# aleflabo/MoCoDAD

Hardware: AMD Instinct MI355X
Metric: pose-clips/sec (whole node) @ noise_steps=10, 5 seeds; AUC vs ref (higher is better)
Workload: dtype f32

## Files before the change

### mocodad_amd/csrc/mcd_api.hip

```cpp

#include <algorithm>
#include "mcd_launch.hpp"
#include "mcd_generic_kernel.hpp"
#include "mcd_pack.hpp"

#if MCD_NWAVES != 8 && !defined(MCD_FAST_T)
#error "mcd_api.hip is built with the default wave count: per-unit wave counts belong to mcd_inst.hip (MCD_UNIT_FLAGS_<n>)"
#endif
namespace { constexpr int API_THREADS = 512; }
#pragma GCC poison NWAVES NTHREADS

using namespace mcd;

#include "mcd_post_kernel.hpp"

namespace {

int launch_score(const mcd_weights* w, int T, ScoreParams& P, hipStream_t st, bool* fused = nullptr, bool layer_test = false) {
    if (!layer_test) {
        P.force_split = w->opt[MCD_OPT_SPLIT];
        P.phase = w->opt[MCD_OPT_PHASE];
        const int variant = w->opt[MCD_OPT_VARIANT];
        if (variant != 0 && !score_has_variants()) return fail(MCD_EUNSUPPORTED, "MCD_OPT_VARIANT needs a -DMCD_TUNING_VARIANTS build");
#define MCD_CASE(unit, V, T_, NB, MINW) if (T == T_ && variant == V) return launch_score_t<T_, NB, MINW>(P, st, fused);
        MCD_SCORE_VARIANT_INSTANCES(MCD_CASE)
#undef MCD_CASE
    }
    switch (layer_test ? -T : T) {
#define MCD_CASE(unit, T_, NB, MINW, LT) case (LT ? -T_ : T_): return launch_score_t<T_, NB, MINW, LT>(P, st, fused);
        MCD_SCORE_INSTANCES(MCD_CASE)
#undef MCD_CASE
        default: break;
    }
    if (layer_test) return fail(MCD_EUNSUPPORTED, "mcd_layer_forward: no layer-test kernel for " + std::to_string(T) + " U-Net frames (the LT rows of mcd_instances.hpp)");
    return fail(MCD_EUNSUPPORTED, "U-Net frame count " + std::to_string(T) + " not instantiated (MCD_SCORE_INSTANCES, mcd_instances.hpp)");
}

#define MCD_COND_CASE(fn, unit, T, NB) case T: return fn<T, NB>(w, data, fi, seg_len, emb, B, st);
int launch_cond_fast(const mcd_weights* w, const DataView& data, const FrameIdx& fi, int seg_len, float* emb, int B, hipStream_t st) {
    switch (w->cond.Tc) {
#define MCD_CASE(unit, T, NB) MCD_COND_CASE(launch_cond_fast_t, unit, T, NB)
        MCD_COND_FAST_INSTANCES(MCD_CASE)
#undef MCD_CASE
        default: break;
    }
    return fail(MCD_EUNSUPPORTED, "cond_fast: frame count not instantiated");
}
int launch_cond_unet(const mcd_weights* w, const DataView& data, const FrameIdx& fi, int seg_len, float* emb, int B, hipStream_t st) {
    switch (w->cond.Tc) {
#define MCD_CASE(unit, T, NB) MCD_COND_CASE(launch_cond_unet_t, unit, T, NB)
        MCD_COND_UNET_INSTANCES(MCD_CASE)
#undef MCD_CASE
        default: break;
    }
    return fail(MCD_EUNSUPPORTED, "E_unet condition encoder: frame count not instantiated");
}
constexpr int GEN_MAX_WGS = 2048;
int64_t gen_scratch_bytes(int64_t units, int T) {
    const int64_t wgs = units < GEN_MAX_WGS ? units : GEN_MAX_WGS;
    return wgs * (int64_t)GEN_SLAB * T * 4;
}
int launch_score_generic(const mcd_weights* w, const ScoreParams& P, const FrameMaps& M, float* scratch, hipStream_t st) {
    const int T = w->cfg.t_unet;
    const int wgs = P.n_chains < GEN_MAX_WGS ? P.n_chains : GEN_MAX_WGS;
    const size_t lds = ((size_t)3 * C0 * T * 17 + EMB_TOTAL + 4 + EDIM + GEN_THREADS) * 4;
    hipLaunchKernelGGL(score_generic_kernel, dim3(wgs), dim3(GEN_THREADS), lds, st, P, M, w->gen, T, scratch);
    HIP_TRY(hipGetLastError());
    return MCD_OK;
}
int tiled_wgs(const mcd_weights* w, int64_t chains, int TP) {
    int cus = 256;
    (void)hipDeviceGetAttribute(&cus, hipDeviceAttributeMultiprocessorCount, w->device);
    if (cus < 1) cus = 256;
    const int64_t units = (chains + tl_nb(TP) - 1) / tl_nb(TP);
    cus *= tl_wgs_per_cu(TP);
    return (int)(units < cus ? units : cus);
}
int64_t tiled_scratch_bytes(const mcd_weights* w, int64_t chains, int TP) { return (int64_t)tiled_wgs(w, chains, TP) * tl_slab_floats(TP * tl_nb(TP)) * 4; }
int launch_score_tiled(const mcd_weights* w, const ScoreParams& P, const FrameMaps& M, float* scratch, hipStream_t st, bool layer_test = false) {
    int dev = -1;
    HIP_TRY(hipGetDevice(&dev));
    if (dev != w->device) return fail(MCD_EINVAL, "the current device is not the handle's device (the workspace slabs are sized for it)");
    const int wgs = tiled_wgs(w, P.n_chains, w->tiled_tp);
    switch (layer_test ? -w->tiled_tp : w->tiled_tp) {
#define MCD_CASE(unit, TP, NB, LT) case (LT ? -TP : TP): return launch_score_tiled_t<TP, NB, LT>(w, P, M, scratch, wgs, st);
        MCD_TILED_INSTANCES(MCD_CASE)
#undef MCD_CASE
        default: return fail(MCD_EUNSUPPORTED, "tiled kernel: frame count");
    }
}
constexpr int CE_MAX_WGS = 512;
int launch_cond_plain(const mcd_weights* w, const float* cond_data, int B, float* emb, float* scratch, hipStream_t st) {
    const bool g = w->cond.gmode != 0;
    if (g && !scratch) return fail(MCD_EINVAL, "workspace required (mcd_score_workspace_bytes) for this many condition frames");
    const size_t lds = ((size_t)(g ? 2 : 3) * w->cond.cmax * w->cond.Tc * 17 + CE_THREADS) * 4;
    LDS_LIMIT(&cond_encode_kernel, (size_t)160 * 1024);
    const int wgs = g && B > CE_MAX_WGS ? CE_MAX_WGS : B;
    hipLaunchKernelGGL(cond_encode_kernel, dim3(wgs), dim3(CE_THREADS), lds, st, w->cond, cond_data, emb, B, g ? scratch : nullptr);
    HIP_TRY(hipGetLastError());
    return MCD_OK;
}
enum UnetRoute { UNET_KERNEL, UNET_TILED, UNET_GENERIC };
UnetRoute unet_route(const mcd_weights* w, bool honour_option = true) {
    if (honour_option && w->opt[MCD_OPT_GENERIC_UNET]) return UNET_GENERIC;
    return w->fast_unet ? UNET_KERNEL : w->tiled_tp ? UNET_TILED : UNET_GENERIC;
}
enum CondRoute {
    COND_NONE,
    COND_INKERNEL,
    COND_FAST,
    COND_UNET,
    COND_TILED,
    COND_UNET_GENERIC,
    COND_PLAIN,
    COND_PLAIN_SCRATCH
};
CondRoute cond_route(const mcd_weights* w, bool whole_windows = false) {
    if (!w->has_cond) return COND_NONE;
    const bool generic = w->opt[MCD_OPT_COND_GENERIC] != 0;
    if (w->cond_unet) {
        if (generic) return COND_UNET_GENERIC;
        return cond_unet_has_kernel(w->cond.Tc) ? COND_UNET : w->tiled_cond_tp ? COND_TILED : COND_UNET_GENERIC;
    }
    if (w->cond_fast && !generic) return whole_windows ? COND_INKERNEL : COND_FAST;
    return w->cond.gmode ? COND_PLAIN_SCRATCH : COND_PLAIN;
}
int64_t unet_scratch_bytes(const mcd_weights* w, UnetRoute r, int64_t chains) {
    switch (r) {
        case UNET_TILED: return w->tiled_tp ? tiled_scratch_bytes(w, chains, w->tiled_tp) : 0;
        case UNET_GENERIC: return gen_scratch_bytes(chains, w->cfg.t_unet);
        default: return 0;
    }
}
int64_t cond_scratch_bytes(const mcd_weights* w, CondRoute r, int64_t B) {
    switch (r) {
        case COND_TILED: return w->cond_unet && w->tiled_cond_tp ? tiled_scratch_bytes(w, B, w->tiled_cond_tp) : 0;
        case COND_UNET_GENERIC: return w->cond_unet ? gen_scratch_bytes(B, w->cond.Tc) : 0;
        case COND_PLAIN_SCRATCH:
            return w->has_cond && !w->cond_unet && w->cond.gmode ? (B < CE_MAX_WGS ? B : CE_MAX_WGS) * (int64_t)w->cond.cmax * w->cond.Tc * 17 * 4 : 0;
        default: return 0;
    }
}
int64_t unet_ws_bytes(const mcd_weights* w, int64_t chains) {
    if (!w->fast_unet) return std::max(unet_scratch_bytes(w, UNET_TILED, chains), unet_scratch_bytes(w, UNET_GENERIC, chains));
    return unet_scratch_bytes(w, unet_route(w), chains);
}
int64_t cond_ws_bytes(const mcd_weights* w, int64_t B) {
    return std::max({cond_scratch_bytes(w, COND_TILED, B), cond_scratch_bytes(w, COND_UNET_GENERIC, B), cond_scratch_bytes(w, COND_PLAIN_SCRATCH, B)});
}

int launch_unet(const mcd_weights* w, UnetRoute r, ScoreParams& P, const FrameMaps& M, float* scratch, hipStream_t st, bool* fused = nullptr) {
    switch (r) {
        case UNET_KERNEL: return launch_score(w, w->cfg.t_unet, P, st, fused);
        case UNET_TILED: return launch_score_tiled(w, P, M, scratch, st);
        default: return launch_score_generic(w, P, M, scratch, st);
    }
}
int launch_cond_view(const mcd_weights* w, CondRoute r, const DataView& data, const FrameIdx& fi, int seg_len, float* emb, int B, float* scratch,
                     hipStream_t st) {
    if (r == COND_FAST) return launch_cond_fast(w, data, fi, seg_len, emb, B, st);
    if (r == COND_UNET) return launch_cond_unet(w, data, fi, seg_len, emb, B, st);
    const int Tc = w->cond.Tc;
    if (!scratch) return fail(MCD_EINVAL, "workspace required (mcd_score_workspace_bytes) for the runtime-shape condition encoder");
    if (r == COND_TILED) {
        ScoreParams P;
        memset(&P, 0, sizeof(P));
        P.wbuf = w->dbuf; P.dv = data; P.seg_len = seg_len; P.B = B; P.S = 1; P.n_chains = B; P.ns = 2; P.eps_out = emb;
        FrameMaps M;
        memset(&M, 0, sizeof(M));
        for (int t = 0; t < Tc; ++t) M.src_frame[t] = fi.idx[t];
        const int wgs = tiled_wgs(w, B, w->tiled_cond_tp);
        switch (w->tiled_cond_tp) {
#define MCD_CASE(unit, TP, NB) case TP: return launch_score_tiled_t<TP, NB, false, true>(w, P, M, scratch, wgs, st);
            MCD_TILED_COND_INSTANCES(MCD_CASE)
#undef MCD_CASE
            default: return fail(MCD_EUNSUPPORTED, "tiled condition encoder: frame count");
        }
    }
    const int wgs = B < GEN_MAX_WGS ? B : GEN_MAX_WGS;
    hipLaunchKernelGGL(cond_unet_generic_kernel, dim3(wgs), dim3(GEN_THREADS), 0, st, w->dbuf, w->gcond, data, fi, seg_len, Tc, B, emb, scratch);
    HIP_TRY(hipGetLastError());
    return MCD_OK;
}
int upload_packed(const std::vector<float>& buf, int device, float** dbuf, int** tune = nullptr) {
    int prev_dev = 0;
    HIP_TRY(hipGetDevice(&prev_dev));
    HIP_TRY(hipSetDevice(device));
    struct Restore { int d; ~Restore() { (void)hipSetDevice(d); } } restore{prev_dev};
    *dbuf = nullptr;
    hipError_t e = hipMalloc(reinterpret_cast<void**>(dbuf), buf.size() * sizeof(float));
    if (e != hipSuccess) return fail(MCD_EDEVICE, std::string("hipMalloc: ") + hipGetErrorString(e));
    e = hipMemcpy(*dbuf, buf.data(), buf.size() * sizeof(float), hipMemcpyHostToDevice);
    if (e != hipSuccess) { (void)hipFree(*dbuf); return fail(MCD_EDEVICE, std::string("hipMemcpy: ") + hipGetErrorString(e)); }
    if (tune) {
        *tune = nullptr;
        if (hipMalloc(reinterpret_cast<void**>(tune), 4 * sizeof(int)) != hipSuccess || hipMemset(*tune, 0, 4 * sizeof(int)) != hipSuccess) {
            if (*tune) (void)hipFree(*tune);
            (void)hipFree(*dbuf);
            return fail(MCD_EDEVICE, "hipMalloc (tuning words)");
        }
    }
    return MCD_OK;
}
}

#include "mcd_call.hpp"

static unsigned long long* g_prof = nullptr;

#pragma GCC visibility push(default)
extern "C" {

void mcd_debug_set_prof(void* p) { g_prof = reinterpret_cast<unsigned long long*>(p); }

int mcd_debug_poison_lds(void* stream) {
    constexpr size_t lds = 160 * 1024;
    LDS_LIMIT(poison_lds_kernel, lds);
    hipLaunchKernelGGL(poison_lds_kernel, dim3(4096), dim3(API_THREADS), lds, static_cast<hipStream_t>(stream), (unsigned*)nullptr, (int)(lds / 4));
    HIP_TRY(hipGetLastError());
    return MCD_OK;
}

const char* mcd_last_error(void) { return g_err.c_str(); }
int32_t mcd_abi_version(void) { return MCD_ABI_VERSION; }

int mcd_pack_weights(const mcd_tensor_t* tensors, int32_t n_tensors, const mcd_model_cfg_t* cfg, int32_t device,
                     mcd_weights_t** out) {
    if (!tensors || !cfg || !out) return fail(MCD_EINVAL, "null argument");
    PackedModel m;
    int rc = pack_pose_model(tensors, n_tensors, cfg, m);
    if (rc != MCD_OK) return rc;
    float* dbuf = nullptr;
    int* tune = nullptr;
    rc = upload_packed(m.buf, device, &dbuf, &tune);
    if (rc != MCD_OK) return rc;
    mcd_weights* w = new mcd_weights();
    memset(w->opt, 0, sizeof(w->opt));
    w->cfg = *cfg; w->device = device; w->dbuf = dbuf; w->tune = tune; w->n_floats = m.buf.size();
    w->zero_row = m.zero_row; w->fast_unet = m.fast_unet != 0; w->gen = m.gen; w->tiled = m.tiled; w->tiled_tp = m.tiled_tp;
    w->gcond = m.cond.GC; w->tiled_cond = m.cond.TNc; w->tiled_cond_tp = m.cond.tiled_cond_tp;
    set_cond_weights(w, m, dbuf);
    *out = w;
    return MCD_OK;
}

int mcd_debug_pack_digest(const mcd_tensor_t* tensors, int32_t n_tensors, const mcd_model_cfg_t* cfg, const mcd_latent_cfg_t* latent_cfg,
                          int64_t* n_floats_out, uint64_t* digest_out) {
    if (!tensors || !cfg || !n_floats_out || !digest_out) return fail(MCD_EINVAL, "null argument");
    PackedModel m;
    const int rc = latent_cfg ? pack_latent_model(tensors, n_tensors, cfg, latent_cfg, m) : pack_pose_model(tensors, n_tensors, cfg, m);
    if (rc != MCD_OK) return rc;
    *n_floats_out = (int64_t)m.buf.size();
    *digest_out = pack_digest(m);
    return MCD_OK;
}

int mcd_set_option(mcd_weights_t* w, int32_t option, int32_t value) {
    if (!w) return fail(MCD_EINVAL, "null argument");
    if (option < 0 || option >= MCD_OPT_COUNT) return fail(MCD_EINVAL, "unknown option " + std::to_string(option));
    w->opt[option] = value;
    return MCD_OK;
}

void mcd_free_weights(mcd_weights_t* w) {
    if (!w) return;
    if (w->dbuf) (void)hipFree(w->dbuf);
    if (w->tune) (void)hipFree(w->tune);
    delete w;
}

int mcd_cond_encode(const mcd_weights_t* w, const float* cond_data, int32_t n_windows, float* emb_out, void* stream) {
    if (!w) return fail(MCD_EINVAL, "null argument");
    if (!w->has_cond) return fail(MCD_EINVAL, "model has no condition encoder");
    if (n_windows <= 0) return MCD_OK;
    if (!cond_data || !emb_out) return fail(MCD_EINVAL, "null argument");
    const CondRoute route = cond_route(w);
    if (w->cond_unet && !cond_unet_has_kernel(w->cond.Tc))
        return fail(MCD_EUNSUPPORTED, "mcd_cond_encode: the 'E_unet' encoder at this frame count needs scratch memory; use mcd_score");
    if (route == COND_PLAIN_SCRATCH) return fail(MCD_EUNSUPPORTED, "mcd_cond_encode: this many condition frames need scratch memory; use mcd_score");
    FrameIdx fi;
    for (int k = 0; k < MCD_MAX_FRAMES; ++k) fi.idx[k] = k;
    DataView dv;
    window_view(cond_data, nullptr, w->cond.Tc, dv);
    return launch_cond(w, route, dv, fi, w->cond.Tc, emb_out, n_windows, nullptr, nullptr, (hipStream_t)stream);
}

int64_t mcd_pass_workspace_bytes(const mcd_weights_t* w, int32_t n_windows) {
    if (!w || n_windows <= 0) return 0;
    return unet_ws_bytes(w, n_windows);
}

int mcd_unet_forward(const mcd_weights_t* w, const float* x, const float* cond, const float* step_table, int32_t t,
                     int32_t n_windows, float* eps_out, void* workspace, void* stream) {
    if (!w) return fail(MCD_EINVAL, "null argument");
    if (n_windows <= 0) return MCD_OK;
    if (!x || !step_table || !eps_out) return fail(MCD_EINVAL, "null argument");
    if (t < 0) return fail(MCD_EINVAL, "t must be >= 0 (step_table needs at least t + 1 rows)");
    ScoreParams P;
    memset(&P, 0, sizeof(P));
    P.wbuf = w->dbuf; P.x_in = x; P.cond_emb = cond; P.step_table = step_table; P.eps_out = eps_out;
    P.B = n_windows; P.S = 1; P.ns = t + 1; P.seg_len = w->cfg.t_unet; P.n_corrupt = w->cfg.t_unet; P.fixed_mask = 0;
    P.mode = 1; P.step_single = t; P.n_chains = n_windows;
    hipStream_t st = (hipStream_t)stream;
    const UnetRoute route = unet_route(w);
    if (route != UNET_KERNEL && !workspace) return fail(MCD_EINVAL, "workspace required (mcd_pass_workspace_bytes)");
    FrameMaps M;
    memset(&M, 0, sizeof(M));
    return launch_unet(w, route, P, M, reinterpret_cast<float*>(workspace), st);
}

int mcd_layer_forward(const mcd_weights_t* w, int32_t stage, const float* x, const float* skip, const float* emb, int32_t n_windows,
                      float* out, void* workspace, void* stream) {
    if (!w) return fail(MCD_EINVAL, "null argument");
    if (stage < 0 || stage > 14) return fail(MCD_EINVAL, "stage must be 0..10 (ST-GCN layers) or 11..14 (down1, down2, up3, up2)");
    if (n_windows <= 0) return MCD_OK;
    if (!x || !out || !emb) return fail(MCD_EINVAL, "null argument");
    ScoreParams P;
    memset(&P, 0, sizeof(P));
    P.wbuf = w->dbuf; P.cond_emb = emb; P.step_table = w->dbuf + w->zero_row;
    P.B = n_windows; P.S = 1; P.ns = 1; P.seg_len = w->cfg.t_unet; P.n_corrupt = w->cfg.t_unet;
    P.mode = 1; P.step_single = 0; P.n_chains = n_windows;
    P.lt_stage = stage; P.lt_in = x; P.lt_out = out; P.lt_skip = skip;
    P.x_in = stage == 0 ? x : nullptr;
    hipStream_t st = (hipStream_t)stream;
    if (unet_route(w, false) == UNET_TILED) {
        if (stage > 10) return fail(MCD_EUNSUPPORTED, "13 .. 32 U-Net frames: the joint resamplers are part of stages 3, 5, 7, 9");
        if (skip && stage != 7 && stage != 9) return fail(MCD_EINVAL, "skip tensor: stages 7 (d2) and 9 (d1) only");
        if (!workspace) return fail(MCD_EINVAL, "workspace required (mcd_pass_workspace_bytes)");
        FrameMaps M;
        memset(&M, 0, sizeof(M));
        return launch_score_tiled(w, P, M, reinterpret_cast<float*>(workspace), st, true);
    }
    if (skip) return fail(MCD_EINVAL, "skip tensor: only the fused stages of 13 .. 32 U-Net frames take one");
    return launch_score(w, w->cfg.t_unet, P, st, nullptr, true);
}

int mcd_philox_noise(uint64_t seed, int64_t first_window_id, int32_t n_windows, int32_t n_samples, int32_t noise_steps,
                     int32_t n_corrupt, float* noise_out, void* stream) {
    if (n_windows <= 0) return MCD_OK;
    if (!noise_out) return fail(MCD_EINVAL, "null argument");
    if (n_samples < 1 || noise_steps < 2 || n_corrupt < 1 || n_corrupt > MCD_MAX_FRAMES) return fail(MCD_EINVAL, "bad sizes");
    const int K = noise_steps > 2 ? noise_steps - 1 : 1;
    const long long total = (long long)n_samples * K * n_windows * n_corrupt * 9;
    hipLaunchKernelGGL(philox_noise_kernel, dim3((unsigned)((total + 255) / 256)), dim3(256), 0, (hipStream_t)stream,
                       (unsigned long long)seed, (long long)first_window_id, n_windows, n_samples, K, n_corrupt, noise_out);
    HIP_TRY(hipGetLastError());
    return MCD_OK;
}

int mcd_random_imp_masks(uint64_t seed, int64_t first_window_id, int32_t n_windows, int32_t seg_len, int32_t n_cond,
                         int32_t* mask_out, void* stream) {
    if (seg_len < 2 || seg_len > MCD_MAX_FRAMES) return fail(MCD_EINVAL, "seg_len must be in 2 .. 32 (one mask bit per frame)");
    if (n_cond < 1 || n_cond >= seg_len) return fail(MCD_EINVAL, "n_cond must be in 1 .. seg_len - 1");
    if (n_windows < 0) return fail(MCD_EINVAL, "n_windows must be >= 0");
    if (n_windows == 0) return MCD_OK;
    if (!mask_out) return fail(MCD_EINVAL, "mask_out is null");
    hipLaunchKernelGGL(random_imp_masks_kernel, dim3((unsigned)((n_windows + 255) / 256)), dim3(256), 0, (hipStream_t)stream,
                       (unsigned long long)seed, (long long)first_window_id, n_windows, seg_len, n_cond, mask_out);
    HIP_TRY(hipGetLastError());
    return MCD_OK;
}

int32_t mcd_plan_split(const mcd_weights_t* w, const mcd_score_cfg_t* cfg) {
    if (!w || !cfg) return fail(MCD_EINVAL, "null argument");
    if (cfg->n_windows <= 0) return 1;
    if (unet_route(w) != UNET_KERNEL) return 0;
    ScoreParams P;
    memset(&P, 0, sizeof(P));
    P.B = cfg->n_windows; P.S = cfg->n_samples; P.ns = cfg->noise_steps; P.mode = 0; P.plan_only = 1;
    const int rc = launch_score(w, w->cfg.t_unet, P, nullptr);
    return rc != MCD_OK ? rc : P.split;
}

int64_t mcd_score_workspace_bytes(const mcd_weights_t* w, const mcd_score_cfg_t* cfg) {
    if (!w || !cfg) return 0;
    return pose_workspace(w, cfg->n_windows, cfg->n_samples).bytes;
}

static int launch_aggregate(AggrParams& A, hipStream_t st) {
    A.in_lds = A.S <= AGG_LDS_MAX;
    const size_t lds = (size_t)(2 + (A.in_lds ? A.S : 0)) * sizeof(float);
    hipLaunchKernelGGL(aggregate_kernel, dim3(A.B < 65536 ? A.B : 65536), dim3(64), lds, st, A);
    HIP_TRY(hipGetLastError());
    return MCD_OK;
}

static int score_impl(const mcd_weights_t* w, const mcd_score_cfg_t* cfg, const float* data, const mcd_window_view_t* view,
                      const float* noise, uint64_t seed, int64_t first_window_id, const float* step_table, void* workspace,
                      int aggr, float quantile, float* loss_agg, float* loss_all, float* pose_out, void* stream) {
    if (!w || !cfg) return fail(MCD_EINVAL, "null argument");
    const int B = cfg->n_windows, S = cfg->n_samples;
    if (B <= 0) return MCD_OK;
    if (!data || !step_table) return fail(MCD_EINVAL, "null argument");
    if (aggr == 0 && !loss_all) return fail(MCD_EINVAL, "null argument");
    if (aggr != 0) {
        if (!loss_agg) return fail(MCD_EINVAL, "null argument");
        if (int rc = check_aggregation(aggr, quantile, AGGR_LOSSES, "mcd_score_fused aggregates losses (best, worst, mean, median, quantile); "
                                                                    "the *_pose strategies go through mcd_score + mcd_aggregate")) return rc;
    }
    if (S < 1 || cfg->noise_steps < 2) return fail(MCD_EINVAL, "need n_samples >= 1 and noise_steps >= 2");
    if ((long long)B * S > 0x7fffffffll) return fail(MCD_EINVAL, "n_windows x n_samples exceeds 2^31 - 1: score in smaller batches");
    if (int rc = check_frame_partition(cfg)) return rc;
    const int strat = w->cfg.strategy;
    const int Tu = w->cfg.t_unet;
    const bool rnd = strat == MCD_STRATEGY_RANDOM_IMP;
    const bool keeps_cond = strat == MCD_STRATEGY_CONCAT || strat == MCD_STRATEGY_INBETWEEN_IMP || rnd;
    if (rnd && !(view && view->cond_mask)) return fail(MCD_EINVAL, "random_imp needs mcd_window_view_t.cond_mask");
    const int tf = keeps_cond ? cfg->n_cond : 0;
    if (tf + cfg->n_corrupt != Tu) return fail(MCD_EINVAL, "frame split does not match the packed U-Net (t_unet)");
    const UnetRoute route = unet_route(w);
    if (strat == MCD_STRATEGY_INJECT && cfg->n_cond != w->cfg.t_cond) return fail(MCD_EINVAL, "n_cond does not match the packed condition encoder");
    hipStream_t st = (hipStream_t)stream;
    ScoreParams P;
    memset(&P, 0, sizeof(P));
    P.wbuf = w->dbuf; P.prof = g_prof;
    P.tune = w->opt[MCD_OPT_PHASE] == -2 ? nullptr : w->tune;
    if (int rc = window_view(data, view, cfg->seg_len, P.dv)) return rc;
    if (rnd) P.win_mask = view->cond_mask;
    P.noise = noise; P.step_table = step_table; P.pose_out = pose_out;
    P.seed = seed; P.first_window = first_window_id;
    P.B = B; P.S = S; P.ns = cfg->noise_steps; P.seg_len = cfg->seg_len; P.n_corrupt = cfg->n_corrupt;
    P.loss_fn = cfg->loss_fn; P.mode = 0; P.n_chains = B * S; P.split = 1;
    P.aggr = aggr; P.aggr_q = quantile; P.loss_agg = aggr ? loss_agg : nullptr;
    FrameMaps M;
    memset(&M, 0, sizeof(M));
    if (int rc = check_frame_lists(cfg)) return rc;
    for (int k = 0; k < tf && !rnd; ++k) {
        const int t = strat == MCD_STRATEGY_INBETWEEN_IMP ? cfg->cond_idx[k] : k;
        if (t < 0 || t >= Tu || ((P.fixed_mask >> t) & 1)) return fail(MCD_EINVAL, "bad cond_idx");
        P.fixed_mask |= 1u << t;
        M.src_frame[t] = cfg->cond_idx[k];
    }
    for (int k = 0; k < cfg->n_corrupt && !rnd; ++k) {
        const int t = strat == MCD_STRATEGY_INBETWEEN_IMP ? cfg->corrupt_idx[k] : tf + k;
        if (t < 0 || t >= Tu || ((P.fixed_mask >> t) & 1)) return fail(MCD_EINVAL, "bad corrupt_idx");
        M.src_frame[t] = cfg->corrupt_idx[k];
        M.tx_of[t] = k;
        M.pos_of[k] = t;
    }
    for (int t = 0; t < MCD_MAX_FRAMES; ++t) M.upd_of[t] = -1;
    for (int k = 0; k < cfg->n_corrupt && !rnd; ++k) {
        const int t = keeps_cond ? cfg->corrupt_idx[k] : k;
        if (t < 0 || t >= Tu || M.upd_of[t] >= 0) return fail(MCD_EINVAL, "bad corrupt_idx");
        M.upd_of[t] = k;
        if (M.pos_of[k] != t) P.upd_shift = 1;
    }
    for (int t = 0; t < 12; ++t) {
        P.src_frame[t] = M.src_frame[t]; P.tx_of[t] = M.tx_of[t]; P.pos_of[t] = M.pos_of[t]; P.upd_of[t] = M.upd_of[t];
    }
    const PoseWorkspace lay = pose_workspace(w, B, S);
    char* wsb = reinterpret_cast<char*>(workspace);
    float* ws_loss = wsb ? reinterpret_cast<float*>(wsb + lay.loss) : nullptr;
    float* gen_scratch = wsb ? reinterpret_cast<float*>(wsb + lay.scratch) : nullptr;
    P.loss_out = loss_all ? loss_all : ws_loss;
    if (route == UNET_KERNEL) {
        P.plan_only = 1;
        const int rc = launch_score(w, Tu, P, st);
        if (rc != MCD_OK) return rc;
        P.plan_only = 0;
    }
    auto score = [&]() -> int {
        bool fused = false;
        if (route == UNET_KERNEL) P.loss_out_optional = loss_all == nullptr;
        else if (!workspace) return fail(MCD_EINVAL, "workspace required (mcd_score_workspace_bytes) for the runtime-shape kernel");
        const int rc = launch_unet(w, route, P, M, gen_scratch, st, &fused);
        if (rc != MCD_OK || aggr == 0 || fused) return rc;
        AggrParams A;
        memset(&A, 0, sizeof(A));
        A.loss_all = P.loss_out; A.loss_agg = loss_agg; A.B = B; A.S = S; A.C = C0; A.Tx = cfg->n_corrupt; A.V = 17;
        A.seg_len = cfg->seg_len; A.strategy = aggr; A.loss_fn = cfg->loss_fn; A.q = quantile;
        return launch_aggregate(A, st);
    };
    const CondRoute croute = cond_route(w, route == UNET_KERNEL && P.split == 1 && cfg->n_cond == Tu);
    if (croute == COND_INKERNEL) {
        P.cond_inkernel = 1;
        for (int k = 0; k < Tu; ++k) P.cond_idx[k] = cfg->cond_idx[k];
    } else if (croute != COND_NONE) {
        if (!workspace) return fail(MCD_EINVAL, "workspace required for this condition encoder");
        float* emb = reinterpret_cast<float*>(workspace);
        FrameIdx fi;
        for (int k = 0; k < MCD_MAX_FRAMES; ++k) fi.idx[k] = cfg->cond_idx[k];
        if (int rc = launch_cond(w, croute, P.dv, fi, cfg->seg_len, emb, B, reinterpret_cast<float*>(wsb + lay.gather), gen_scratch, st)) return rc;
        P.cond_emb = emb;
    }
    return score();
}

int mcd_score(const mcd_weights_t* w, const mcd_score_cfg_t* cfg, const float* data, const float* noise, uint64_t seed,
              int64_t first_window_id, const float* step_table, void* workspace, float* loss_out, float* pose_out,
              void* stream) {
    return score_impl(w, cfg, data, nullptr, noise, seed, first_window_id, step_table, workspace, 0, 0.f, nullptr, loss_out, pose_out, stream);
}

int mcd_score_view(const mcd_weights_t* w, const mcd_score_cfg_t* cfg, const float* data, const mcd_window_view_t* view,
                   const float* noise, uint64_t seed, int64_t first_window_id, const float* step_table, void* workspace,
                   float* loss_out, float* pose_out, void* stream) {
    return score_impl(w, cfg, data, view, noise, seed, first_window_id, step_table, workspace, 0, 0.f, nullptr, loss_out, pose_out, stream);
}

int mcd_score_fused(const mcd_weights_t* w, const mcd_score_cfg_t* cfg, const float* data, const mcd_window_view_t* view,
                    const float* noise, uint64_t seed, int64_t first_window_id, const float* step_table, void* workspace,
                    int32_t aggregation, float quantile, float* loss_agg, float* loss_all, float* pose_out, void* stream) {
    if (aggregation == MCD_AGGR_ALL) return fail(MCD_EINVAL, "MCD_AGGR_ALL is mcd_score");
    return score_impl(w, cfg, data, view, noise, seed, first_window_id, step_table, workspace, aggregation, quantile, loss_agg, loss_all,
                      pose_out, stream);
}

int mcd_aggregate(const mcd_score_cfg_t* cfg, int32_t num_coords, int32_t n_joints, int32_t strategy, float quantile,
                  const float* loss_all, const float* pose_all, const float* data, float* loss_agg, float* pose_agg,
                  void* stream) {
    return mcd_aggregate_view(cfg, num_coords, n_joints, strategy, quantile, loss_all, pose_all, data, nullptr, loss_agg, pose_agg, stream);
}

int mcd_aggregate_view(const mcd_score_cfg_t* cfg, int32_t num_coords, int32_t n_joints, int32_t strategy, float quantile,
                       const float* loss_all, const float* pose_all, const float* data, const mcd_window_view_t* view,
                       float* loss_agg, float* pose_agg, void* stream) {
    if (!cfg) return fail(MCD_EINVAL, "null argument");
    if (cfg->n_windows <= 0) return MCD_OK;
    if (!loss_all || !loss_agg) return fail(MCD_EINVAL, "null argument");
    if (cfg->n_samples < 1) return fail(MCD_EINVAL, "need n_samples >= 1");
    if (int rc = check_aggregation(strategy, quantile, AGGR_ANY, "unknown aggregation strategy")) return rc;
    const bool need_pose = strategy == MCD_AGGR_MEAN_POSE || strategy == MCD_AGGR_MEDIAN_POSE;
    if (need_pose && (!pose_all || !data)) return fail(MCD_EINVAL, "pose strategies need pose_all and data");
    if (pose_agg && !pose_all) return fail(MCD_EINVAL, "pose_agg requested without pose_all");
    if (cfg->n_windows <= 0) return MCD_OK;
    if (view && view->base) return fail(MCD_EINVAL, "mcd_aggregate_view reads dense (B,C,T,V) windows: materialise the view (base must be NULL)");
    const int32_t* win_mask = view ? view->cond_mask : nullptr;
    if (win_mask && (cfg->seg_len < 1 || cfg->seg_len > MCD_MAX_FRAMES || cfg->n_corrupt < 1 || cfg->n_corrupt > cfg->seg_len))
        return fail(MCD_EINVAL, "cond_mask: need 1 <= n_corrupt <= seg_len <= 32");
    AggrParams P;
    memset(&P, 0, sizeof(P));
    P.loss_all = loss_all; P.pose_all = pose_all; P.data = data; P.loss_agg = loss_agg; P.pose_agg = pose_agg;
    P.B = cfg->n_windows; P.S = cfg->n_samples; P.C = num_coords; P.Tx = cfg->n_corrupt; P.V = n_joints;
    P.seg_len = cfg->seg_len; P.strategy = strategy; P.loss_fn = cfg->loss_fn; P.q = quantile;
    for (int t = 0; t < cfg->n_corrupt && t < MCD_MAX_FRAMES; ++t) P.corrupt_idx[t] = cfg->corrupt_idx[t];
    P.win_mask = win_mask;
    return launch_aggregate(P, (hipStream_t)stream);
}

int mcd_scatter_max(const float* scores, const int32_t* frames, const int32_t* row, int64_t n, int32_t seg_len,
                    int32_t n_rows, int32_t n_frames, float* out, void* stream) {
    if (!scores || !frames || !row || !out) return fail(MCD_EINVAL, "null argument");
    hipStream_t st = (hipStream_t)stream;
    HIP_TRY(hipMemsetAsync(out, 0, (size_t)n_rows * n_frames * sizeof(float), st));
    if (n <= 0) return MCD_OK;
    const long long total = (long long)n * seg_len;
    hipLaunchKernelGGL(scatter_max_kernel, dim3((unsigned)((total + 255) / 256)), dim3(256), 0, st, scores, frames, row,
                       (long long)n, seg_len, n_frames, out);
    HIP_TRY(hipGetLastError());
    return MCD_OK;
}

int mcd_normalize_poses(const float* raw, int64_t n_frames, float vid_w, float vid_h, const double* center,
                        const double* scale, float* out, void* stream) {
    if (n_frames < 0) return fail(MCD_EINVAL, "n_frames < 0");
    if (!std::isfinite(vid_w) || !std::isfinite(vid_h)) return fail(MCD_EINVAL, "vid_res must be finite");
    if (!center != !scale) return fail(MCD_EINVAL, "center and scale are both given or both NULL");
    if (n_frames == 0) return MCD_OK;
    if (!raw || !out) return fail(MCD_EINVAL, "null argument");
    const long long blocks = (n_frames + 255) / 256;
    if (blocks > 0x7fffffffll) return fail(MCD_EUNSUPPORTED, "too many frames for one launch");
    hipLaunchKernelGGL(normalize_poses_kernel, dim3((unsigned)blocks), dim3(256), 0, (hipStream_t)stream, raw,
                       (long long)n_frames, vid_w, vid_h, center, scale, out);
    HIP_TRY(hipGetLastError());
    return MCD_OK;
}

static int stream_params(const mcd_stream_state_t* s, StreamParams* P) {
    if (!s || !s->ring || !s->frame_scores) return fail(MCD_EINVAL, "null stream state");
    if (s->n_slots <= 0 || s->num_transform <= 0 || s->seg_len <= 0 || s->seg_len > MCD_MAX_FRAMES || s->ring_len < s->seg_len)
        return fail(MCD_EINVAL, "stream state: need n_slots, num_transform >= 1 and 1 <= seg_len <= ring_len (seg_len <= 32)");
    if ((int64_t)s->n_slots * 2 * s->ring_len > 0x7fffffffll / 34 || (int64_t)s->n_slots * s->num_transform * s->ring_len > 0x7fffffffll)
        return fail(MCD_EUNSUPPORTED, "stream rings of more than 2^31 elements");
    P->ring = s->ring; P->fs = s->frame_scores;
    P->n_slots = s->n_slots; P->L = s->ring_len; P->seg_len = s->seg_len; P->nt = s->num_transform;
    return MCD_OK;
}

int mcd_stream_push(const mcd_stream_state_t* s, const float* raw, const int32_t* desc, int32_t n, int32_t n_emit,
                    float vid_w, float vid_h, const double* center, const double* scale, int64_t* base_out,
                    int32_t* trans_out, void* stream) {
    StreamParams P;
    if (int rc = stream_params(s, &P)) return rc;
    if (n < 0 || n_emit < 0 || n_emit > n) return fail(MCD_EINVAL, "need 0 <= n_emit <= n");
    if (n > s->n_slots) return fail(MCD_EINVAL, "more rows than slots: a tick holds at most one row per track");
    if (!std::isfinite(vid_w) || !std::isfinite(vid_h)) return fail(MCD_EINVAL, "vid_res must be finite");
    if (!center != !scale) return fail(MCD_EINVAL, "center and scale are both given or both NULL");
    if (n == 0) return MCD_OK;
    if (!raw || !desc || (n_emit > 0 && (!base_out || !trans_out))) return fail(MCD_EINVAL, "null argument");
    hipLaunchKernelGGL(stream_push_kernel, dim3((unsigned)((n + 255) / 256)), dim3(256), 0, (hipStream_t)stream, P, raw, desc, n,
                       n_emit, vid_w, vid_h, center, scale, reinterpret_cast<long long*>(base_out), trans_out);
    HIP_TRY(hipGetLastError());
    return MCD_OK;
}

int mcd_stream_frame_scores(const mcd_stream_state_t* s, const float* scores, const int32_t* win, int32_t n_emit,
                            float* final_out, void* stream) {
    StreamParams P;
    if (int rc = stream_params(s, &P)) return rc;
    if (n_emit < 0 || n_emit > s->n_slots) return fail(MCD_EINVAL, "need 0 <= n_emit <= n_slots");
    if (n_emit == 0) return MCD_OK;
    if (!scores || !win || !final_out) return fail(MCD_EINVAL, "null argument");
    const long long total = (long long)n_emit * P.nt;
    if (total > 0x7fffffffll) return fail(MCD_EUNSUPPORTED, "too many windows for one launch");
    hipLaunchKernelGGL(stream_frame_scores_kernel, dim3((unsigned)((total + 255) / 256)), dim3(256), 0, (hipStream_t)stream, P,
                       scores, win, n_emit, final_out);
    HIP_TRY(hipGetLastError());
    return MCD_OK;
}

int mcd_stream_flush(const mcd_stream_state_t* s, const int32_t* win, int32_t n, float* out, void* stream) {
    StreamParams P;
    if (int rc = stream_params(s, &P)) return rc;
    if (n < 0 || n > s->n_slots) return fail(MCD_EINVAL, "need 0 <= n <= n_slots");
    const long long total = (long long)n * (P.seg_len - 1) * P.nt;
    if (total == 0) return MCD_OK;
    if (!win || !out) return fail(MCD_EINVAL, "null argument");
    if (total > 0x7fffffffll) return fail(MCD_EUNSUPPORTED, "too many tracks for one launch");
    hipLaunchKernelGGL(stream_flush_kernel, dim3((unsigned)((total + 255) / 256)), dim3(256), 0, (hipStream_t)stream, P, win, n, out);
    HIP_TRY(hipGetLastError());
    return MCD_OK;
}


int64_t mcd_frame_scores_workspace_bytes(const mcd_frame_cfg_t* c) {
    if (!c || c->n_clips <= 0 || c->num_transform <= 0 || c->n_persons <= 0 || c->max_frames <= 0) return 0;
    const int64_t rows = (int64_t)c->num_transform * c->n_clips * c->n_persons;
    return rows * c->max_frames * 4 + round256(rows * 4);
}

int mcd_frame_scores(const mcd_frame_cfg_t* c, const float* scores, const int64_t* trans, const int64_t* meta,
                     const int32_t* frames, int64_t n_windows, int32_t seg_len, void* workspace, double* out, void* stream) {
    if (!c || !workspace || !out) return fail(MCD_EINVAL, "null argument");
    if (c->n_clips <= 0 || c->num_transform <= 0 || c->n_persons <= 0 || c->max_frames <= 0) return fail(MCD_EINVAL, "bad sizes");
    if (!c->clip_keys || !c->clip_n_frames || !c->frame_dst || !c->clip_out_len || !c->clip_out_off || !c->gauss_weights)
        return fail(MCD_EINVAL, "null table");
    if (n_windows > 0 && (!scores || !trans || !meta || !frames)) return fail(MCD_EINVAL, "null argument");
    if (c->frames_shift < 1) return fail(MCD_EINVAL, "frames_shift must be >= 1 (the reference's score[:-shift] is empty for 0)");
    if (c->gauss_radius < 0) return fail(MCD_EINVAL, "bad gauss_radius");
    const size_t lds = (size_t)2 * c->max_frames * sizeof(double);
    if (lds > 150 * 1024) return fail(MCD_EUNSUPPORTED, "clips longer than 9600 frames");
    hipStream_t st = (hipStream_t)stream;
    const int64_t rows = (int64_t)c->num_transform * c->n_clips * c->n_persons;
    FrameParams Q;
    memset(&Q, 0, sizeof(Q));
    Q.scores = scores; Q.trans = reinterpret_cast<const long long*>(trans); Q.meta = reinterpret_cast<const long long*>(meta);
    Q.frames = frames; Q.clip_keys = reinterpret_cast<const long long*>(c->clip_keys); Q.clip_n = c->clip_n_frames;
    Q.dst = c->frame_dst; Q.out_len = c->clip_out_len; Q.out_off = reinterpret_cast<const long long*>(c->clip_out_off);
    Q.gauss = c->gauss_weights;
    Q.mat = reinterpret_cast<float*>(workspace);
    Q.used = reinterpret_cast<int*>(Q.mat + rows * c->max_frames);
    Q.out = out; Q.n = n_windows; Q.seg_len = seg_len; Q.n_clips = c->n_clips; Q.num_transform = c->num_transform;
    Q.P = c->n_persons; Q.F = c->max_frames; Q.pad = c->pad_size; Q.shift = c->frames_shift; Q.radius = c->gauss_radius;
    HIP_TRY(hipMemsetAsync(workspace, 0, (size_t)(rows * c->max_frames * 4 + rows * 4), st));
    if (n_windows > 0) {
        const long long total = (long long)n_windows * seg_len;
        hipLaunchKernelGGL(frame_scatter_kernel, dim3((unsigned)((total + 255) / 256)), dim3(256), 0, st, Q);
        HIP_TRY(hipGetLastError());
    }
    LDS_LIMIT(&frame_scores_kernel, (size_t)150 * 1024);
    hipLaunchKernelGGL(frame_scores_kernel, dim3(c->n_clips), dim3(256), lds, st, Q);
    HIP_TRY(hipGetLastError());
    return MCD_OK;
}

}

#include "mcd_latent_api.hpp"
#pragma GCC visibility pop
```

### mocodad_amd/csrc/mcd_device.hpp

```cpp

#pragma once
#include <hip/hip_runtime.h>
#include <stdint.h>
#include <string.h>
#include <stdlib.h>
#include <math.h>
#include <string>
#include <vector>
#include <unordered_map>
#include <utility>
#include <type_traits>
#include <atomic>

#include "../../include/mocodad_hip.h"

namespace mcd {

typedef float f32x4 __attribute__((ext_vector_type(4)));
typedef float f32x2 __attribute__((ext_vector_type(2)));
typedef const float __attribute__((address_space(4))) cfloat;
typedef const float __attribute__((address_space(1))) gfloat;
typedef const f32x4 __attribute__((address_space(1))) gf32x4;
__device__ __forceinline__ gfloat* as_global(const float* p) { return (gfloat*)p; }
typedef float __attribute__((address_space(3))) lds_float;
typedef f32x4 __attribute__((address_space(3))) lds_f32x4;
__device__ __forceinline__ unsigned lds_addr(const float* p) { return (unsigned)(uintptr_t)p; }
__device__ __forceinline__ float4 lds_load4(unsigned addr) {
    const f32x4 v = *(lds_f32x4*)(uintptr_t)addr;
    return make_float4(v[0], v[1], v[2], v[3]);
}
__device__ __forceinline__ void lds_store4(unsigned addr, float a, float b, float c, float d) {
    *(lds_f32x4*)(uintptr_t)addr = f32x4{a, b, c, d};
}
typedef f32x4 __attribute__((address_space(1))) gf32x4_rw;
__device__ __forceinline__ void store_global4(float* p, float4 v) {
    *(gf32x4_rw*)p = f32x4{v.x, v.y, v.z, v.w};
}
__device__ __forceinline__ float4 load_global4(const float* p) {
    const f32x4 v = *(gf32x4*)p;
    return make_float4(v[0], v[1], v[2], v[3]);
}

#ifndef MCD_NWAVES
#define MCD_NWAVES 8
#endif
constexpr int NWAVES = MCD_NWAVES;
constexpr int NTHREADS = NWAVES * 64;
constexpr int C0 = 2;
constexpr int EDIM = 16;
constexpr int NLAYERS = 11;
constexpr int EMB_TOTAL = 532;
constexpr int EMB_STRIDE = 536;

__host__ __device__ constexpr int cs_of(int c) { return c + 4; }
__host__ __device__ constexpr int ceil16(int x) { return (x + 15) / 16 * 16; }

struct LDesc { int cin, cout, V, res; };
__host__ __device__ constexpr LDesc layer_desc(int l) {
    return l == 0 ? LDesc{16, 16, 17, 1}  : l == 1 ? LDesc{16, 32, 17, 1} : l == 2 ? LDesc{32, 32, 17, 0}
         : l == 3 ? LDesc{32, 64, 12, 1} : l == 4 ? LDesc{64, 64, 12, 0} : l == 5 ? LDesc{64, 128, 10, 1}
         : l == 6 ? LDesc{128, 64, 10, 1} : l == 7 ? LDesc{64, 64, 12, 0} : l == 8 ? LDesc{64, 32, 12, 1}
         : l == 9 ? LDesc{32, 32, 17, 0} : LDesc{32, 2, 17, 1};
}
__host__ __device__ constexpr int emb_off(int l) {
    return l == 0 ? 0 : l == 1 ? 16 : l == 2 ? 48 : l == 3 ? 80 : l == 4 ? 144 : l == 5 ? 208 : l == 6 ? 336
         : l == 7 ? 400 : l == 8 ? 464 : l == 9 ? 496 : 528;
}

constexpr int TAB_FLOATS = 256;
enum { F_TQ = 0, F_AM = 1, F_WP = 2, F_BIAS = 3, F_SLOPE = 4, F_STRIDE = 8 };
constexpr int TAB_WE = 88, TAB_BE = 89;
constexpr int TAB_RSW = 90, TAB_RSB = 94;
typedef const int __attribute__((address_space(4))) cint;
__device__ __forceinline__ int tab_i(const float* base, int idx) { return ((cint*)base)[idx]; }
__device__ __forceinline__ float tab_f(const float* base, int idx) { return ((cfloat*)base)[idx]; }
struct LayerW { int tq, am, wp, bias; float slope; };
__device__ __forceinline__ LayerW layer_w(const float* base, int l) {
    LayerW w;
    w.tq = tab_i(base, l * F_STRIDE + F_TQ); w.am = tab_i(base, l * F_STRIDE + F_AM);
    w.wp = tab_i(base, l * F_STRIDE + F_WP); w.bias = tab_i(base, l * F_STRIDE + F_BIAS);
    w.slope = tab_f(base, l * F_STRIDE + F_SLOPE);
    return w;
}

#ifdef MCD_PROFILE
constexpr int PROF_STAGE = 72;
constexpr int PROF_BAR = 30;
constexpr int PROF_NW = NWAVES;
constexpr int PROF_SLOTS = PROF_STAGE + PROF_NW + PROF_BAR * PROF_NW;
constexpr int PROF_TRACE = 128;
#endif
struct Prof {
#ifdef MCD_PROFILE
    unsigned* acc;
    unsigned long long tlast;
    bool on;
    bool won;
    int bidx;
    int wv;
    unsigned* tr;
    bool tr_on;
    __device__ __forceinline__ void trace(int slot) {
        if (tr_on) tr[slot * PROF_NW + wv] = (unsigned)__builtin_readcyclecounter();
    }
    __device__ __forceinline__ void mark(int id) {
        if (on) {
            const unsigned long long t = __builtin_readcyclecounter();
            __hip_atomic_fetch_add(acc + id, (unsigned)(t - tlast), __ATOMIC_RELAXED, __HIP_MEMORY_SCOPE_WORKGROUP);
            tlast = t;
        }
    }
    __device__ __forceinline__ void sync() {
        const unsigned long long t0 = __builtin_readcyclecounter();
        __syncthreads();
        const unsigned long long t1 = __builtin_readcyclecounter();
        if (won && bidx < PROF_BAR)
            __hip_atomic_fetch_add(acc + PROF_STAGE + PROF_NW + bidx * PROF_NW + wv, (unsigned)(t1 - t0), __ATOMIC_RELAXED, __HIP_MEMORY_SCOPE_WORKGROUP);
        ++bidx;
    }
    __device__ __forceinline__ void off() { on = false; won = false; acc = nullptr; tlast = 0; bidx = 0; wv = 0; tr = nullptr; tr_on = false; }
#else
    __device__ __forceinline__ void trace(int) {}
    __device__ __forceinline__ void mark(int) {}
    __device__ __forceinline__ void sync() { __syncthreads(); }
    __device__ __forceinline__ void off() {}
#endif
};
#define bsync() prof.sync()
#define STAGE(id) prof.mark(id)

struct DataView {
    const float* data;
    const long long* base;
    long long sc, st;
    const int* trans;
    const float* aff;
};
__device__ __forceinline__ float load_coord(const DataView& dv, int b, int c, int t, int v, int seg_len) {
    const long long sc = dv.base ? dv.sc : (long long)seg_len * 17;
    const long long st = dv.base ? dv.st : 17;
    const float* p = dv.data + (dv.base ? dv.base[b] : (long long)b * C0 * seg_len * 17) + t * st + v;
    if (!dv.trans) return p[c * sc];
    const float x = p[0], y = p[sc];
    const float* a = dv.aff + dv.trans[b] * 6 + c * 3;
    return (a[0] * x + a[1] * y) + a[2];
}

struct ScoreParams {
    unsigned long long* prof;
    const float* wbuf;
    DataView dv;
    const float* noise;
    const float* cond_emb;
    const float* step_table;
    const float* x_in;
    float* loss_out;
    float* pose_out;
    float* eps_out;
    unsigned long long seed;
    long long first_window;
    int B, S, ns, seg_len, n_corrupt, loss_fn, mode, step_single, n_chains;
    int split, aggr, cond_inkernel;
    int force_split;
    int loss_out_optional;
    int plan_only;
    int phase;
    int prio_shift;
    int prio_rounds;
    int* tune;
    float aggr_q;
    float* loss_agg;
    int cond_idx[12];
    int upd_shift;
    unsigned fixed_mask;
    int src_frame[12];
    int tx_of[12];
    int pos_of[12];
    int upd_of[12];
    const int* win_mask;
    int lt_stage;
    const float* lt_in;
    float* lt_out;
    const float* lt_skip;
};
__device__ __forceinline__ int fm_tx(const ScoreParams& P, int fixed, int t) {
    return P.win_mask ? __popc(~fixed & ((1 << t) - 1)) : P.tx_of[t];
}
__device__ __forceinline__ int fm_src(const ScoreParams& P, int t) { return P.win_mask ? t : P.src_frame[t]; }

__device__ __forceinline__ void philox_normal4(unsigned long long seed, unsigned c0, unsigned c1, unsigned c2, unsigned c3,
                                               float (&z)[4]) {
    unsigned k0 = (unsigned)seed, k1 = (unsigned)(seed >> 32);
#pragma unroll
    for (int r = 0; r < 10; ++r) {
        const unsigned long long p0 = (unsigned long long)0xD2511F53u * c0;
        const unsigned long long p1 = (unsigned long long)0xCD9E8D57u * c2;
        const unsigned n0 = (unsigned)(p1 >> 32) ^ c1 ^ k0;
        const unsigned n1 = (unsigned)p1;
        const unsigned n2 = (unsigned)(p0 >> 32) ^ c3 ^ k1;
        const unsigned n3 = (unsigned)p0;
        c0 = n0; c1 = n1; c2 = n2; c3 = n3;
        k0 += 0x9E3779B9u; k1 += 0xBB67AE85u;
    }
    const unsigned w[4] = {c0, c1, c2, c3};
#pragma unroll
    for (int h = 0; h < 2; ++h) {
        const float u1 = ((float)(w[2 * h] >> 8) + 0.5f) * (1.0f / 16777216.0f);
        const float u2 = ((float)(w[2 * h + 1] >> 8) + 0.5f) * (1.0f / 16777216.0f);
        const float r = __fsqrt_rn(-1.38629436111989f * __log2f(u1));
        z[2 * h] = r * __cosf(6.28318530717958647692f * u2);
        z[2 * h + 1] = r * __sinf(6.28318530717958647692f * u2);
    }
}
__device__ __forceinline__ float philox_normal(unsigned long long seed, unsigned c0, unsigned c1, unsigned c2, unsigned c3) {
    unsigned k0 = (unsigned)seed, k1 = (unsigned)(seed >> 32);
#pragma unroll
    for (int r = 0; r < 10; ++r) {
        const unsigned long long p0 = (unsigned long long)0xD2511F53u * c0;
        const unsigned long long p1 = (unsigned long long)0xCD9E8D57u * c2;
        const unsigned n0 = (unsigned)(p1 >> 32) ^ c1 ^ k0;
        const unsigned n1 = (unsigned)p1;
        const unsigned n2 = (unsigned)(p0 >> 32) ^ c3 ^ k1;
        const unsigned n3 = (unsigned)p0;
        c0 = n0; c1 = n1; c2 = n2; c3 = n3;
        k0 += 0x9E3779B9u; k1 += 0xBB67AE85u;
    }
    const float u1 = ((float)(c0 >> 8) + 0.5f) * (1.0f / 16777216.0f);
    const float u2 = ((float)(c1 >> 8) + 0.5f) * (1.0f / 16777216.0f);
    return __fsqrt_rn(-1.38629436111989f * __log2f(u1)) * __cosf(6.28318530717958647692f * u2);
}
__device__ __forceinline__ void philox_words4(unsigned long long seed, unsigned c0, unsigned c1, unsigned c2, unsigned c3,
                                              unsigned (&w)[4]) {
    unsigned k0 = (unsigned)seed, k1 = (unsigned)(seed >> 32);
#pragma unroll
    for (int r = 0; r < 10; ++r) {
        const unsigned long long p0 = (unsigned long long)0xD2511F53u * c0;
        const unsigned long long p1 = (unsigned long long)0xCD9E8D57u * c2;
        const unsigned n0 = (unsigned)(p1 >> 32) ^ c1 ^ k0;
        const unsigned n1 = (unsigned)p1;
        const unsigned n2 = (unsigned)(p0 >> 32) ^ c3 ^ k1;
        const unsigned n3 = (unsigned)p0;
        c0 = n0; c1 = n1; c2 = n2; c3 = n3;
        k0 += 0x9E3779B9u; k1 += 0xBB67AE85u;
    }
    w[0] = c0; w[1] = c1; w[2] = c2; w[3] = c3;
}
__device__ __forceinline__ int nth_set_bit(unsigned m, int r) {
    for (int i = 0; i < r; ++i) m &= m - 1u;
    return __ffs(m) - 1;
}
__device__ __forceinline__ unsigned low_bits(int n) { return n >= 32 ? 0xFFFFFFFFu : (1u << n) - 1u; }

__device__ __forceinline__ float prelu_bound(float a) {
    return __int_as_float(__float_as_int(a) <= 0x3f800000 ? 0x7f800000 : (int)0xff800000);
}
__device__ __forceinline__ float prelu(float x, float a) { return __builtin_amdgcn_fmed3f(x, a * x, prelu_bound(a)); }

template <int CTRL>
__device__ __forceinline__ float dpp_f(float v) {
    return __int_as_float(__builtin_amdgcn_update_dpp(0, __float_as_int(v), CTRL, 0xf, 0xf, true));
}
__device__ __forceinline__ float row16_sum(float v) {
    v += dpp_f<0xB1>(v);
    v += dpp_f<0x4E>(v);
    v += dpp_f<0x141>(v);
    v += dpp_f<0x140>(v);
    return v;
}

__device__ __forceinline__ float aggregate_losses(float* L, int S, int strategy, float q) {
    if (strategy == MCD_AGGR_BEST || strategy == MCD_AGGR_WORST) {
        const bool best = strategy == MCD_AGGR_BEST;
        float cur = best ? 1e10f : -1.f;
        for (int s = 0; s < S; ++s) if (best ? (L[s] < cur) : (L[s] > cur)) cur = L[s];
        return cur;
    }
    if (strategy == MCD_AGGR_MEAN) {
        float sum = 0.f;
        for (int s = 0; s < S; ++s) sum += L[s];
        return sum / (float)S;
    }
    for (int s = 0; s < S; ++s)
        if (L[s] != L[s]) return L[s];
    for (int i = 1; i < S; ++i) {
        const float x = L[i];
        int k = i - 1;
        while (k >= 0 && L[k] > x) { L[k + 1] = L[k]; --k; }
        L[k + 1] = x;
    }
    if (strategy == MCD_AGGR_MEDIAN) return L[(S - 1) / 2];
    const float pos = fminf(fmaxf(q, 0.f), 1.f) * (float)(S - 1);
    const int lo = (int)floorf(pos);
    const int hi = lo + 1 < S ? lo + 1 : S - 1;
    const float wgt = pos - (float)lo;
    const float a = L[lo], c = L[hi];
    return wgt < 0.5f ? a + wgt * (c - a) : c - (c - a) * (1.f - wgt);
}

template <int L, bool PAD = false>
__device__ __forceinline__ void fmac_bc(float& acc, float coef, float y) {
    if (PAD)
        asm("v_fmac_f32_dpp %0, %1, %2 row_newbcast:%3 row_mask:0xf bank_mask:0xf\n\ts_nop 1" : "+v"(acc) : "v"(coef), "v"(y), "n"(L));
    else
        asm("v_fmac_f32_dpp %0, %1, %2 row_newbcast:%3 row_mask:0xf bank_mask:0xf" : "+v"(acc) : "v"(coef), "v"(y), "n"(L));
}
template <int L, bool PAD = false>
__device__ __forceinline__ float mul_bc(float coef, float y) {
    float r;
    if (PAD)
        asm("v_mul_f32_dpp %0, %1, %2 row_newbcast:%3 row_mask:0xf bank_mask:0xf\n\ts_nop 1" : "=v"(r) : "v"(coef), "v"(y), "n"(L));
    else
        asm("v_mul_f32_dpp %0, %1, %2 row_newbcast:%3 row_mask:0xf bank_mask:0xf" : "=v"(r) : "v"(coef), "v"(y), "n"(L));
    return r;
}
#define MCD_DPP(OP, I) OP " %[y" #I "], %[c" #I "], %[x] row_newbcast:%[L] row_mask:0xf bank_mask:0xf\n\t"
#define MCD_TM_IN(I) [c##I] "v"(c[I])
#define MCD_TM2(OP, CON, NOP) asm(MCD_DPP(OP, 0) MCD_DPP(OP, 1) NOP : [y0] CON(y[0]), [y1] CON(y[1]) \
                                  : MCD_TM_IN(0), MCD_TM_IN(1), [x] "v"(x), [L] "n"(L))
#define MCD_TM3(OP, CON, NOP) asm(MCD_DPP(OP, 0) MCD_DPP(OP, 1) MCD_DPP(OP, 2) NOP : [y0] CON(y[0]), [y1] CON(y[1]), [y2] CON(y[2]) \
                                  : MCD_TM_IN(0), MCD_TM_IN(1), MCD_TM_IN(2), [x] "v"(x), [L] "n"(L))
#define MCD_TM4(OP, CON, NOP) asm(MCD_DPP(OP, 0) MCD_DPP(OP, 1) MCD_DPP(OP, 2) MCD_DPP(OP, 3) NOP \
                                  : [y0] CON(y[0]), [y1] CON(y[1]), [y2] CON(y[2]), [y3] CON(y[3]) \
                                  : MCD_TM_IN(0), MCD_TM_IN(1), MCD_TM_IN(2), MCD_TM_IN(3), [x] "v"(x), [L] "n"(L))
#define MCD_TM5(OP, CON, NOP) asm(MCD_DPP(OP, 0) MCD_DPP(OP, 1) MCD_DPP(OP, 2) MCD_DPP(OP, 3) MCD_DPP(OP, 4) NOP \
                                  : [y0] CON(y[0]), [y1] CON(y[1]), [y2] CON(y[2]), [y3] CON(y[3]), [y4] CON(y[4]) \
                                  : MCD_TM_IN(0), MCD_TM_IN(1), MCD_TM_IN(2), MCD_TM_IN(3), MCD_TM_IN(4), [x] "v"(x), [L] "n"(L))
#define MCD_TM6(OP, CON, NOP) asm(MCD_DPP(OP, 0) MCD_DPP(OP, 1) MCD_DPP(OP, 2) MCD_DPP(OP, 3) MCD_DPP(OP, 4) MCD_DPP(OP, 5) NOP \
                                  : [y0] CON(y[0]), [y1] CON(y[1]), [y2] CON(y[2]), [y3] CON(y[3]), [y4] CON(y[4]), [y5] CON(y[5]) \
                                  : MCD_TM_IN(0), MCD_TM_IN(1), MCD_TM_IN(2), MCD_TM_IN(3), MCD_TM_IN(4), MCD_TM_IN(5), [x] "v"(x), [L] "n"(L))
#define MCD_TM(N) do { if constexpr (INIT) { if constexpr (PAD) MCD_TM##N("v_mul_f32_dpp", "=&v", "s_nop 1"); else MCD_TM##N("v_mul_f32_dpp", "=&v", ""); } \
                       else { if constexpr (PAD) MCD_TM##N("v_fmac_f32_dpp", "+v", "s_nop 1"); else MCD_TM##N("v_fmac_f32_dpp", "+v", ""); } } while (0)
template <int QC, int L, bool INIT, bool PAD>
__device__ __forceinline__ void tm_step(float (&y)[QC], const float (&c)[QC], float x) {
    static_assert(QC >= 1 && QC <= 6, "time-mix group sizes");
    if constexpr (QC == 1) {
        if constexpr (INIT) y[0] = mul_bc<L, PAD>(c[0], x);
        else fmac_bc<L, PAD>(y[0], c[0], x);
    } else if constexpr (QC == 2) {
        MCD_TM(2);
    } else if constexpr (QC == 3) {
        MCD_TM(3);
    } else if constexpr (QC == 4) {
        MCD_TM(4);
    } else if constexpr (QC == 5) {
        MCD_TM(5);
    } else {
        MCD_TM(6);
    }
}
template <int... Is, class F>
__device__ __forceinline__ void static_for_impl(std::integer_sequence<int, Is...>, F&& f) {
    (f(std::integral_constant<int, Is>{}), ...);
}
template <int N, class F>
__device__ __forceinline__ void static_for(F&& f) { static_for_impl(std::make_integer_sequence<int, N>{}, f); }

constexpr int MIX_QPAD = 4;

__host__ __device__ constexpr int mix_vmap(int V, int ks, int g) {
    return ks < 2 * (((V + 3) / 4) / 2) ? 8 * (ks >> 1) + 2 * (ks & 1) + 4 * (g & 1) + (g >> 1) : 8 * (((V + 3) / 4) / 2) + g;
}

template <int CIN, int V, int T, int NB>
struct MixCfg {
    static constexpr int KS = (V + 3) / 4;
    static constexpr int KP = 2 * (KS / 2);
    static constexpr int MT = (V + 15) / 16;
    static constexpr int CB = CIN / 16;
    static constexpr int QALL = (T % 3 == 0) ? 3 : (T % 2 == 0) ? 2 : T == 5 ? 3 : (T == 7 || T == 11) ? 4 : 1;
    static constexpr int Q2 = (T % 2 == 0 || T == 5 || T == 7 || T == 11) ? 2 : 1;
    static constexpr int units_of(int qc) { return NB * CB * ((T + qc - 1) / qc); }
    static constexpr int Q6 = (T == 12) ? 6 : 1;
    static constexpr int Q5 = (T == 10) ? 5 : 1, Q4 = (T == 8) ? 4 : 1;
    static constexpr int measured_qc() {
        if (NB == 1 && NWAVES == 12 && T >= 7) return CIN >= 64 ? (T == 10 && CIN == 64 ? 5 : T >= 10 ? 4 : 3) : CIN == 32 ? 2 : 1;
        if (NB != 1 || NWAVES != 8) return 0;
        if (CIN == 32 && (T == 5 || T == 9 || T == 10 || T == 11)) return 3;
        if (CIN == 16 && T == 9) return 2;
        return 0;
    }
    static constexpr int QX = measured_qc();
    static constexpr int QC = QX > 0 ? QX : (Q6 > 1 && units_of(Q6) >= NWAVES) ? Q6 : (Q5 > 1 && units_of(Q5) >= NWAVES) ? Q5
                            : (Q4 > 1 && units_of(Q4) >= NWAVES) ? Q4 : units_of(QALL) >= NWAVES ? QALL : units_of(Q2) >= NWAVES ? Q2
                            : 2 * units_of(QALL) > NWAVES ? QALL : 2 * units_of(Q2) > NWAVES ? Q2 : 1;
    static constexpr int NQ = (T + QC - 1) / QC;
    static constexpr bool RAGGED = NQ * QC != T;
    static_assert(NQ * QC - T < MIX_QPAD, "zero rows behind the coefficient tables");
    static constexpr int UNITS = NB * CB * NQ;
    static constexpr int PER = (UNITS + NWAVES - 1) / NWAVES;
    static constexpr int NR = (KS * T + 15) / 16;
    static constexpr bool SAMEQ = NQ == 3 && UNITS == 12 && NWAVES == 8;
    static_assert(T > 12 || PER == 1 || UNITS % NWAVES == 0 || SAMEQ, "mix units: a partial round of units (see MixCfg::QX)");
    __device__ static __forceinline__ int unit_of(int wave, int round) {
        if constexpr (SAMEQ) {
            if (wave < 4) return (wave >> 1) + NQ * ((wave & 1) * 2 + round);
            return round == 0 ? 2 + NQ * (wave - 4) : -1;
        } else {
            const int u = wave + round * NWAVES;
            return u < UNITS ? u : -1;
        }
    }
};
template <int CIN, int V, int T, int NB>
struct MixCoef {
    using M = MixCfg<CIN, V, T, NB>;
    float tq[M::QC][M::NR], aop[M::QC][M::MT][M::KS];
    __device__ __forceinline__ void load(const float* tqd, const float* af, int wave, int lane) {
        load_unit(tqd, af, M::unit_of(wave, 0), lane);
    }
    __device__ __forceinline__ void load_unit(const float* tqd, const float* af, int u, int lane) {
        gfloat* tqd_g = as_global(tqd);
        gfloat* af_g = as_global(af);
        const int uc = u < 0 ? 0 : (u < M::UNITS ? u : M::UNITS - 1);
        const int q0 = (uc % M::NQ) * M::QC;
#pragma unroll
        for (int qi = 0; qi < M::QC; ++qi) {
#pragma unroll
            for (int r = 0; r < M::NR; ++r) tq[qi][r] = tqd_g[((q0 + qi) * M::NR + r) * 64 + lane];
#pragma unroll
            for (int mt = 0; mt < M::MT; ++mt)
#pragma unroll
                for (int ks = 0; ks < M::KS; ++ks) aop[qi][mt][ks] = af_g[(((q0 + qi) * M::MT + mt) * M::KS + ks) * 64 + lane];
        }
    }
};

struct ChIdx {
    int cb16, j;
    __device__ __forceinline__ operator int() const { return cb16 + j; }
};
struct ZeroInit { __device__ __forceinline__ float operator()(int, int, int, int) const { return 0.f; } };
template <int CIN, int V, int T, int NB, bool FORCE = false, bool SCORE = false, class Init, class Store>
__device__ __forceinline__ void mix_stage(const float* __restrict__ in, int cs_in, const MixCoef<CIN, V, T, NB>& pre,
                                          const float* __restrict__ tqd, const float* __restrict__ af, int wave, int lane,
                                          Init&& init, Store&& store) {
    using M = MixCfg<CIN, V, T, NB>;
    constexpr int KS = M::KS, KP = M::KP, MT = M::MT, CB = M::CB, QC = M::QC, NQ = M::NQ, PER = M::PER;
    constexpr bool XB32 = FORCE || SCORE;
    const int j = lane & 15, g = lane >> 4;
    const int voff_pair = 4 * (g & 1) + (g >> 1);
    auto load_x = [&](int u, float (&x)[KS][T]) {
        const int rest = u / NQ;
        const int cb = rest % CB, n = rest / CB;
        unsigned ua = lds_addr(in) + 4u * (unsigned)(n * (T * V) * cs_in + cb * 16);
        asm volatile("" : "+s"(ua));
        const lds_float* ub = (const lds_float*)(uintptr_t)ua;
        const lds_float* a_p = ub + (__mul24(voff_pair, cs_in) + j);
        const lds_float* a_l = (V == 17) ? ub + j : ub + (__mul24(g, cs_in) + j);
        static_for<KS>([&](auto si) {
            constexpr int ks = decltype(si)::value;
            constexpr int vbase = ks < KP ? 8 * (ks >> 1) + 2 * (ks & 1) : 4 * KP;
            const lds_float* xb = ks < KP ? a_p : a_l;
#pragma unroll
            for (int t = 0; t < T; ++t) {
                if constexpr (XB32) x[ks][t] = ((const volatile lds_float*)xb)[(t * V + vbase) * cs_in];
                else x[ks][t] = xb[(t * V + vbase) * cs_in];
            }
        });
    };
    auto unit = [&](const MixCoef<CIN, V, T, NB>& cur, int u, const float (&xs)[KS][T]) {
        const int q0 = (u % NQ) * QC, rest = u / NQ;
        const int cb = rest % CB, n = rest / CB;
        constexpr bool J16 = V == 17;
        constexpr int MTM = J16 ? 1 : MT;
        constexpr bool ZINIT = std::is_same_v<std::decay_t<Init>, ZeroInit>;
        static_assert(ZINIT || !J16, "a seeded accumulator (W-first layers) on a 17-joint layer: joint 16's seed is not wired up");
        f32x4 acc[QC][MTM];
        float part[QC];
#pragma unroll
        for (int qi = 0; qi < QC; ++qi) {
            part[qi] = 0.f;
#pragma unroll
            for (int mt = 0; mt < MTM; ++mt)
                if ((M::RAGGED && q0 + qi >= T) || ZINIT) {
                    acc[qi][mt] = f32x4{0.f, 0.f, 0.f, 0.f};
                } else {
                    acc[qi][mt] = init(n, q0 + qi, mt * 16 + j, ChIdx{cb * 16, 4 * g});
                }
        }
        static_for<KS>([&](auto si) {
            constexpr int ks = decltype(si)::value;
            const float (&x)[T] = xs[ks];
            float y[QC];
            static_for<T>([&](auto ti) {
                constexpr int t = decltype(ti)::value;
                float c[QC];
#pragma unroll
                for (int qi = 0; qi < QC; ++qi) c[qi] = cur.tq[qi][(ks * T + t) / 16];
                tm_step<QC, (ks * T + t) % 16, t == 0, t == T - 1>(y, c, x[t]);
            });
            static_for<QC>([&](auto qq) {
                constexpr int qi = decltype(qq)::value;
#pragma unroll
                for (int mt = 0; mt < MTM; ++mt)
                    acc[qi][mt] = __builtin_amdgcn_mfma_f32_16x16x4f32(y[qi], cur.aop[qi][mt][ks], acc[qi][mt], 0, 0, 0);
                if constexpr (J16) part[qi] = fmaf(cur.aop[qi][1][ks], y[qi], part[qi]);
            });
        });
#pragma unroll
        for (int qi = 0; qi < QC; ++qi) {
            if (M::RAGGED && q0 + qi >= T) continue;
#pragma unroll
            for (int mt = 0; mt < MTM; ++mt) {
                if ((mt + 1) * 16 <= V || mt * 16 + j < V) store(n, q0 + qi, mt * 16 + j, ChIdx{cb * 16, 4 * g}, acc[qi][mt]);
            }
            if constexpr (J16) {
                const unsigned u = __float_as_uint(part[qi]);
                const auto h = __builtin_amdgcn_permlane32_swap(u, u, false, false);
                const unsigned v2 = __float_as_uint(__uint_as_float(h[0]) + __uint_as_float(h[1]));
                const auto f = __builtin_amdgcn_permlane16_swap(v2, v2, false, false);
                const float z16 = __uint_as_float(f[0]) + __uint_as_float(f[1]);
                if (g == 0) store(n, q0 + qi, 16, ChIdx{cb * 16, j}, z16);
            }
        }
    };
    {
        MixCoef<CIN, V, T, NB> cur = pre;
        static_for<PER>([&](auto ri) {
            constexpr int rnd = decltype(ri)::value;
            constexpr bool ALLW = (FORCE || SCORE) && !M::SAMEQ && M::UNITS == PER * NWAVES;
            const int u = ALLW ? wave + rnd * NWAVES : M::unit_of(wave, rnd);
            constexpr bool SURE = ALLW;
            float xs[KS][T];
            load_x(SURE ? u : (u < 0 ? 0 : u), xs);
            if constexpr (FORCE) __builtin_amdgcn_sched_barrier(0);
            MixCoef<CIN, V, T, NB> nxt;
            if constexpr (rnd + 1 < PER && !M::SAMEQ && NQ > 1) nxt.load_unit(tqd, af, M::unit_of(wave, rnd + 1), lane);
            if (SURE || u >= 0) unit(cur, u, xs);
            if constexpr (rnd + 1 < PER && !M::SAMEQ && NQ > 1) cur = nxt;
        });
    }
}
template <int CIN, int V, int T, int NB, class Init, class Store>
__device__ __forceinline__ void mix_stage(const float* __restrict__ in, int cs_in, const float* __restrict__ tqd,
                                          const float* __restrict__ af, int wave, int lane, Init&& init, Store&& store) {
    MixCoef<CIN, V, T, NB> mc;
    mc.load(tqd, af, wave, lane);
    mix_stage<CIN, V, T, NB>(in, cs_in, mc, tqd, af, wave, lane, init, store);
}

template <int C, int VIN, int VOUT, int T, int NB, bool CAPTURE>
struct RsCfg {
    static constexpr int KS = CAPTURE ? (VIN > 16 ? 5 : 4) : (VIN + 3) / 4;
    static constexpr int MT = (VOUT + 15) / 16;
    static constexpr int CB = C / 16;
    static constexpr int UNITS = NB * T * CB;
    static constexpr int PER = (UNITS + NWAVES - 1) / NWAVES;
    static constexpr int VS = CAPTURE ? VIN : VOUT;
    static constexpr int SK = VS > 16 ? 5 : 4;
    static constexpr bool ALIGNED = NB * CB == NWAVES && PER == T;
};
__host__ __device__ constexpr int rs_vmap(bool capture, int vin, int ks, int g) {
    return capture ? (ks < 4 ? 4 * g + ks : 16 + g) : mix_vmap(vin, ks, g);
}

template <int C, int VIN, int VOUT, int T, int NB, bool CAPTURE>
struct RsCoef {
    using RC = RsCfg<C, VIN, VOUT, T, NB, CAPTURE>;
    float aop[RC::MT][RC::KS];
    float bias[RC::MT][4];
    __device__ __forceinline__ void load(const float* wf, const float* bdp, int lane) {
        gfloat* wf_g = as_global(wf);
        gfloat* bdp_g = as_global(bdp);
        const int g = lane >> 4;
#pragma unroll
        for (int mt = 0; mt < RC::MT; ++mt)
#pragma unroll
            for (int ks = 0; ks < RC::KS; ++ks) aop[mt][ks] = wf_g[(mt * RC::KS + ks) * 64 + lane];
#pragma unroll
        for (int mt = 0; mt < RC::MT; ++mt)
#pragma unroll
            for (int r = 0; r < 4; ++r) bias[mt][r] = bdp_g[mt * 16 + 4 * g + r];
    }
};

template <int C, int VIN, int VOUT, int T, int NB, bool CAPTURE, bool ADD, bool ILP = false, bool SQMAP = false, int NSK>
__device__ __forceinline__ void resample_stage(const float* __restrict__ in, int cs_in, float* __restrict__ out, int cs_out,
                                               const RsCoef<C, VIN, VOUT, T, NB, CAPTURE>& rc,
                                               float (&skip)[NSK], int wave, int lane) {
    using RC = RsCfg<C, VIN, VOUT, T, NB, CAPTURE>;
    constexpr int KS = RC::KS, MT = RC::MT, CB = RC::CB, UNITS = RC::UNITS, PER = RC::PER, SK = RC::SK;
    static_assert(!(CAPTURE || ADD) || NSK == PER * SK, "skip register count");
    constexpr int KP = 2 * (((VIN + 3) / 4) / 2);
    const int j = lane & 15, g = lane >> 4;
    const auto& aop = rc.aop;
    const auto& bias = rc.bias;
    float xr[CAPTURE ? 1 : PER][CAPTURE ? 1 : KS] = {};
    constexpr bool FULL = (CAPTURE || ADD) && UNITS == PER * NWAVES;
    using SM = std::conditional_t<SQMAP, MixCfg<(SQMAP ? C : 32), (SQMAP ? (CAPTURE ? VOUT : VIN) : 12), (SQMAP ? T : 3), (SQMAP ? NB : 2)>, MixCfg<32, 12, 3, 2>>;
    static_assert(!SQMAP || (SM::SAMEQ && UNITS == SM::UNITS && PER == SM::PER && !RC::ALIGNED), "SQMAP: the 12-unit SAMEQ mixes only");
    auto unit_at = [&](int i, int& cb, int& nt) -> bool {
        if constexpr (SQMAP) {
            const int um = SM::unit_of(wave, i);
            const int uu = um < 0 ? 0 : um, grp = uu / SM::NQ;
            cb = grp % CB; nt = (grp / CB) * T + uu % SM::NQ;
            return um >= 0;
        } else {
            const int u = wave + i * NWAVES;
            cb = RC::ALIGNED ? wave % CB : u % CB; nt = RC::ALIGNED ? (wave / CB) * T + i : u / CB;
            return FULL || u < UNITS;
        }
    };
    static_for<PER>([&](auto pi) {
        constexpr int i = decltype(pi)::value;
        int cb, nt;
        if (unit_at(i, cb, nt)) {
            const float* ub = in + (nt * VIN * cs_in + cb * 16);
            const float* a_main = ub + (__mul24(CAPTURE ? 4 * g : 4 * (g & 1) + (g >> 1), cs_in) + j);
            const float* a_tail = CAPTURE ? ub + j : ub + (__mul24(g, cs_in) + j);
            static_for<KS>([&](auto si) {
                constexpr int ks = decltype(si)::value;
                constexpr bool MAIN = CAPTURE ? ks < 4 : ks < KP;
                constexpr int row0 = CAPTURE ? (ks < 4 ? ks : 16) : (ks < KP ? 8 * (ks >> 1) + 2 * (ks & 1) : 4 * KP);
                const float xv = (MAIN ? a_main : a_tail)[row0 * cs_in];
                if constexpr (CAPTURE) skip[i * SK + ks] = xv;
                else xr[i][ks] = xv;
            });
        }
    });
    constexpr bool J16 = VOUT == 17;
    constexpr int MTM = J16 ? 1 : MT;
    auto finish = [&](auto pi, f32x4 (&acc)[MTM], float part) {
        constexpr int i = decltype(pi)::value;
        int cb, nt;
        unit_at(i, cb, nt);
        if constexpr (ADD) {
#pragma unroll
            for (int r = 0; r < 4; ++r) acc[0][r] += skip[i * SK + r];
            if constexpr (SK == 5 && !J16) acc[MT - 1][0] += skip[i * SK + 4];
        }
        float* uo = out + (nt * VOUT * cs_out + cb * 16);
        float* zo = uo + (__mul24(4 * g, cs_out) + j);
#pragma unroll
        for (int mt = 0; mt < MTM; ++mt)
#pragma unroll
            for (int r = 0; r < 4; ++r)
                if (mt * 16 + 4 * g + r < VOUT) zo[(mt * 16 + r) * cs_out] = acc[mt][r];
        if constexpr (J16) {
            const unsigned pu = __float_as_uint(part);
            const auto h = __builtin_amdgcn_permlane32_swap(pu, pu, false, false);
            const unsigned v2 = __float_as_uint(__uint_as_float(h[0]) + __uint_as_float(h[1]));
            const auto f = __builtin_amdgcn_permlane16_swap(v2, v2, false, false);
            float z16 = __uint_as_float(f[0]) + __uint_as_float(f[1]) + bias[1][0];
            if constexpr (ADD && SK == 5) z16 += skip[i * SK + 4];
            if (g == 0) uo[16 * cs_out + j] = z16;
        }
    };
    if constexpr (ILP) {
        f32x4 acc[PER][MTM];
        float part[PER];
#pragma unroll
        for (int i = 0; i < PER; ++i) {
            part[i] = 0.f;
#pragma unroll
            for (int mt = 0; mt < MTM; ++mt) acc[i][mt] = f32x4{bias[mt][0], bias[mt][1], bias[mt][2], bias[mt][3]};
        }
        static_for<KS>([&](auto si) {
            constexpr int ks = decltype(si)::value;
            static_for<PER>([&](auto pi) {
                constexpr int i = decltype(pi)::value;
                float x;
                if constexpr (CAPTURE) x = skip[i * SK + ks]; else x = xr[i][ks];
#pragma unroll
                for (int mt = 0; mt < MTM; ++mt) acc[i][mt] = __builtin_amdgcn_mfma_f32_16x16x4f32(aop[mt][ks], x, acc[i][mt], 0, 0, 0);
                if constexpr (J16) part[i] = fmaf(aop[1][ks], x, part[i]);
            });
        });
        static_for<PER>([&](auto pi) {
            int cb_, nt_;
            if (unit_at(decltype(pi)::value, cb_, nt_)) finish(pi, acc[decltype(pi)::value], part[decltype(pi)::value]);
        });
    } else {
        static_for<PER>([&](auto pi) {
            constexpr int i = decltype(pi)::value;
            int cb_, nt_;
            if (unit_at(i, cb_, nt_)) {
                f32x4 acc[MTM];
                float part = 0.f;
#pragma unroll
                for (int mt = 0; mt < MTM; ++mt) acc[mt] = f32x4{bias[mt][0], bias[mt][1], bias[mt][2], bias[mt][3]};
                static_for<KS>([&](auto si) {
                    constexpr int ks = decltype(si)::value;
                    float x;
                    if constexpr (CAPTURE) x = skip[i * SK + ks]; else x = xr[i][ks];
#pragma unroll
                    for (int mt = 0; mt < MTM; ++mt) acc[mt] = __builtin_amdgcn_mfma_f32_16x16x4f32(aop[mt][ks], x, acc[mt], 0, 0, 0);
                    if constexpr (J16) part = fmaf(aop[1][ks], x, part);
                });
                finish(pi, acc, part);
            }
        });
    }
}

__host__ __device__ constexpr int cmax(int a, int b) { return a > b ? a : b; }

template <int MT, int NT>
struct Tiling {
    static constexpr int MW = MT > NWAVES ? MT / NWAVES : 1;
    static constexpr int NG = MT > NWAVES ? 1 : NWAVES / MT;
    static constexpr int MAXN = (NT + NG - 1) / NG;
};
template <int MT, int KQ>
__device__ __forceinline__ void load_afrags(const float4* __restrict__ wp, int wave, int lane, float4 (&a)[KQ], int mi = 0) {
    const float* wpl = reinterpret_cast<const float*>(wp + (((wave + mi * NWAVES) % MT) * KQ) * 64 + lane);
#pragma unroll
    for (int kq = 0; kq < KQ; ++kq) a[kq] = load_global4(wpl + kq * 256);
}

struct NoPre { static constexpr bool none = true; };
template <int MT, int NT, int KQ1, int KQ2, bool IDRES, bool FORCE = false, bool DUAL = FORCE, class Epi, class Pre = NoPre>
__device__ __forceinline__ void gemm_tiles(const float4 (&a)[KQ1 + KQ2], const float* __restrict__ b1, int cs1,
                                           const float* __restrict__ b2, int cs2, int wave, int lane, Epi&& epi, int mi = 0,
                                           const float4 cinit = make_float4(0.f, 0.f, 0.f, 0.f), Pre&& pre = Pre{}) {
    constexpr bool HASPRE = !std::is_same_v<std::decay_t<Pre>, NoPre>;
    constexpr int NG = Tiling<MT, NT>::NG;
    constexpr int MAXN = Tiling<MT, NT>::MAXN;
    const int mt = (wave + mi * NWAVES) % MT, ng = MT > NWAVES ? 0 : wave / MT;
    if (NWAVES % MT != 0 && MT <= NWAVES && ng >= NG) return;
    const int j = lane & 15, g = lane >> 4;
    const int c0 = mt * 16 + 4 * g;
    const int col0 = ng * 16 + j;
    const float* const p1b = b1 + __mul24(col0, cs1) + 4 * g;
    const float* const p2b = b2 + __mul24(col0, cs2) + 4 * g;
    constexpr int KQ = KQ1 + KQ2;
    constexpr int DEPTH0 = KQ < 3 ? KQ : 3;
    auto one_tile = [&](auto ii) {
        constexpr int i = decltype(ii)::value;
        const int col = col0 + i * NG * 16;
        f32x4 c = {cinit.x, cinit.y, cinit.z, cinit.w};
        const float* p1 = p1b + i * NG * 16 * cs1;
        const float* p2 = p2b + i * NG * 16 * cs2;
        if (IDRES) {
            const float4 r = *reinterpret_cast<const float4*>(p2 - 4 * g + c0);
            c[0] = r.x; c[1] = r.y; c[2] = r.z; c[3] = r.w;
        }
        auto rd = [&](auto kk) {
            constexpr int kq = decltype(kk)::value;
            return *reinterpret_cast<const float4*>(kq < KQ1 ? p1 + kq * 16 : p2 + (kq - KQ1) * 16);
        };
        float4 buf[DEPTH0];
        static_for<DEPTH0>([&](auto dd) { buf[decltype(dd)::value] = rd(dd); });
        float4 pe = make_float4(0.f, 0.f, 0.f, 0.f);
        if constexpr (HASPRE) pe = pre(ii, col, ng);
        if constexpr (FORCE) __builtin_amdgcn_sched_barrier(0);
        static_for<KQ>([&](auto kk) {
            constexpr int kq = decltype(kk)::value;
            const float4 u = buf[kq % DEPTH0];
            if constexpr (kq + DEPTH0 < KQ) buf[kq % DEPTH0] = rd(std::integral_constant<int, kq + DEPTH0>{});
            if constexpr (FORCE) __builtin_amdgcn_sched_barrier(0);
            c = __builtin_amdgcn_mfma_f32_16x16x4f32(a[kq].x, u.x, c, 0, 0, 0);
            c = __builtin_amdgcn_mfma_f32_16x16x4f32(a[kq].y, u.y, c, 0, 0, 0);
            c = __builtin_amdgcn_mfma_f32_16x16x4f32(a[kq].z, u.z, c, 0, 0, 0);
            c = __builtin_amdgcn_mfma_f32_16x16x4f32(a[kq].w, u.w, c, 0, 0, 0);
        });
        if constexpr (HASPRE) epi(ii, col, c0, c, col0, ng, pe);
        else epi(ii, col, c0, c, col0, ng);
    };
    auto two_tiles = [&](auto ia, auto ib) {
        constexpr int i0 = decltype(ia)::value, i1 = decltype(ib)::value;
        const float* p1[2] = {p1b + i0 * NG * 16 * cs1, p1b + i1 * NG * 16 * cs1};
        const float* p2[2] = {p2b + i0 * NG * 16 * cs2, p2b + i1 * NG * 16 * cs2};
        f32x4 c[2];
#pragma unroll
        for (int h = 0; h < 2; ++h) {
            c[h] = f32x4{cinit.x, cinit.y, cinit.z, cinit.w};
            if (IDRES) {
                const float4 r = *reinterpret_cast<const float4*>(p2[h] - 4 * g + c0);
                c[h][0] = r.x; c[h][1] = r.y; c[h][2] = r.z; c[h][3] = r.w;
            }
        }
        auto rd = [&](int h, auto kk) {
            constexpr int kq = decltype(kk)::value;
            return *reinterpret_cast<const float4*>(kq < KQ1 ? p1[h] + kq * 16 : p2[h] + (kq - KQ1) * 16);
        };
        float4 buf[2][DEPTH0];
        static_for<DEPTH0>([&](auto dd) { buf[0][decltype(dd)::value] = rd(0, dd); buf[1][decltype(dd)::value] = rd(1, dd); });
        float4 pe0 = make_float4(0.f, 0.f, 0.f, 0.f), pe1 = pe0;
        if constexpr (HASPRE) { pe0 = pre(ia, col0 + i0 * NG * 16, ng); pe1 = pre(ib, col0 + i1 * NG * 16, ng); }
        __builtin_amdgcn_sched_barrier(0);
        static_for<KQ>([&](auto kk) {
            constexpr int kq = decltype(kk)::value;
            const float4 u0 = buf[0][kq % DEPTH0], u1 = buf[1][kq % DEPTH0];
            if constexpr (kq + DEPTH0 < KQ) {
                buf[0][kq % DEPTH0] = rd(0, std::integral_constant<int, kq + DEPTH0>{});
                buf[1][kq % DEPTH0] = rd(1, std::integral_constant<int, kq + DEPTH0>{});
            }
            __builtin_amdgcn_sched_barrier(0);
            c[0] = __builtin_amdgcn_mfma_f32_16x16x4f32(a[kq].x, u0.x, c[0], 0, 0, 0);
            c[1] = __builtin_amdgcn_mfma_f32_16x16x4f32(a[kq].x, u1.x, c[1], 0, 0, 0);
            c[0] = __builtin_amdgcn_mfma_f32_16x16x4f32(a[kq].y, u0.y, c[0], 0, 0, 0);
            c[1] = __builtin_amdgcn_mfma_f32_16x16x4f32(a[kq].y, u1.y, c[1], 0, 0, 0);
            c[0] = __builtin_amdgcn_mfma_f32_16x16x4f32(a[kq].z, u0.z, c[0], 0, 0, 0);
            c[1] = __builtin_amdgcn_mfma_f32_16x16x4f32(a[kq].z, u1.z, c[1], 0, 0, 0);
            c[0] = __builtin_amdgcn_mfma_f32_16x16x4f32(a[kq].w, u0.w, c[0], 0, 0, 0);
            c[1] = __builtin_amdgcn_mfma_f32_16x16x4f32(a[kq].w, u1.w, c[1], 0, 0, 0);
        });
        if constexpr (HASPRE) {
            epi(ia, col0 + i0 * NG * 16, c0, c[0], col0, ng, pe0);
            epi(ib, col0 + i1 * NG * 16, c0, c[1], col0, ng, pe1);
        } else {
            epi(ia, col0 + i0 * NG * 16, c0, c[0], col0, ng);
            epi(ib, col0 + i1 * NG * 16, c0, c[1], col0, ng);
        }
    };
    constexpr bool PIPE = DUAL && MAXN >= 2 && !HASPRE;
    constexpr int PW = DUAL ? 2 : 1;
    constexpr int DEPTH = PIPE ? 1 : DEPTH0;
    if constexpr (PIPE) {
        constexpr int NP = (MAXN + PW - 1) / PW;
        const int nv = (NT - ng + NG - 1) / NG;
        float4 bufs[2][2][DEPTH];
        float4 seed[2][2];
        f32x4 accs[2][2];
        auto rdt = [&](int i, auto kk) {
            constexpr int kq = decltype(kk)::value;
            return *reinterpret_cast<const float4*>(kq < KQ1 ? p1b + i * NG * 16 * cs1 + kq * 16 : p2b + i * NG * 16 * cs2 + (kq - KQ1) * 16);
        };
        auto fetch = [&](auto pp, auto dd) {
            constexpr int p = decltype(pp)::value, d = decltype(dd)::value;
            if constexpr (p < NP) {
                constexpr int i0 = PW * p, i1 = (PW == 2 && i0 + 1 < MAXN) ? i0 + 1 : i0;
                bufs[p & 1][0][d] = rdt(i0, dd);
                if constexpr (i1 != i0) bufs[p & 1][1][d] = rdt(i1, dd);
                if constexpr (IDRES && d == DEPTH - 1 && NWAVES == 12) {
                    seed[p & 1][0] = *reinterpret_cast<const float4*>(p2b + i0 * NG * 16 * cs2 - 4 * g + c0);
                    if constexpr (i1 != i0) seed[p & 1][1] = *reinterpret_cast<const float4*>(p2b + i1 * NG * 16 * cs2 - 4 * g + c0);
                }
            }
        };
        auto epi_pair = [&](auto pp, auto nn) {
            constexpr int p = decltype(pp)::value, N = decltype(nn)::value, i0 = PW * p, i1 = i0 + 1;
            epi(std::integral_constant<int, i0>{}, col0 + i0 * NG * 16, c0, accs[p & 1][0], col0, ng);
            if constexpr (N == 2) epi(std::integral_constant<int, i1>{}, col0 + i1 * NG * 16, c0, accs[p & 1][1], col0, ng);
        };
        auto chain = [&](auto pp, auto nn) {
            constexpr int p = decltype(pp)::value, N = decltype(nn)::value, i0 = PW * p, i1 = N == 2 ? i0 + 1 : i0;
            f32x4 (&c)[2] = accs[p & 1];
#pragma unroll
            for (int h = 0; h < N; ++h) {
                c[h] = f32x4{cinit.x, cinit.y, cinit.z, cinit.w};
                if (IDRES) {
                    if constexpr (NWAVES != 12) seed[p & 1][h] = *reinterpret_cast<const float4*>(p2b + (h ? i1 : i0) * NG * 16 * cs2 - 4 * g + c0);
                    c[h] = f32x4{seed[p & 1][h].x, seed[p & 1][h].y, seed[p & 1][h].z, seed[p & 1][h].w};
                }
            }
            static_for<KQ>([&](auto kk) {
                constexpr int kq = decltype(kk)::value;
                float4 u[2];
#pragma unroll
                for (int h = 0; h < N; ++h) u[h] = bufs[p & 1][h][kq % DEPTH];
                if constexpr (kq + DEPTH < KQ) {
                    bufs[p & 1][0][kq % DEPTH] = rdt(i0, std::integral_constant<int, kq + DEPTH>{});
                    if constexpr (N == 2) bufs[p & 1][1][kq % DEPTH] = rdt(i1, std::integral_constant<int, kq + DEPTH>{});
                } else if constexpr (N == PW) {
                    fetch(std::integral_constant<int, p + 1>{}, std::integral_constant<int, kq + DEPTH - KQ>{});
                }
                __builtin_amdgcn_sched_barrier(0);
                c[0] = __builtin_amdgcn_mfma_f32_16x16x4f32(a[kq].x, u[0].x, c[0], 0, 0, 0);
                if constexpr (N == 2) c[1] = __builtin_amdgcn_mfma_f32_16x16x4f32(a[kq].x, u[1].x, c[1], 0, 0, 0);
                c[0] = __builtin_amdgcn_mfma_f32_16x16x4f32(a[kq].y, u[0].y, c[0], 0, 0, 0);
                if constexpr (N == 2) c[1] = __builtin_amdgcn_mfma_f32_16x16x4f32(a[kq].y, u[1].y, c[1], 0, 0, 0);
                c[0] = __builtin_amdgcn_mfma_f32_16x16x4f32(a[kq].z, u[0].z, c[0], 0, 0, 0);
                if constexpr (N == 2) c[1] = __builtin_amdgcn_mfma_f32_16x16x4f32(a[kq].z, u[1].z, c[1], 0, 0, 0);
                c[0] = __builtin_amdgcn_mfma_f32_16x16x4f32(a[kq].w, u[0].w, c[0], 0, 0, 0);
                if constexpr (N == 2) c[1] = __builtin_amdgcn_mfma_f32_16x16x4f32(a[kq].w, u[1].w, c[1], 0, 0, 0);
                if constexpr (kq == 0 && p > 0) {
                    __builtin_amdgcn_sched_barrier(0);
                    epi_pair(std::integral_constant<int, p - 1>{}, std::integral_constant<int, PW>{});
                    __builtin_amdgcn_sched_barrier(0);
                }
            });
            if (PW * (p + 1) >= nv) epi_pair(pp, nn);
        };
        static_for<DEPTH>([&](auto dd) { fetch(std::integral_constant<int, 0>{}, dd); });
        static_for<NP>([&](auto pp) {
            constexpr int i0 = PW * decltype(pp)::value, i1 = i0 + 1;
            if constexpr (PW == 2 && i1 < MAXN) {
                if (i1 < nv) chain(pp, std::integral_constant<int, 2>{});
                else if (i0 < nv) chain(pp, std::integral_constant<int, 1>{});
            } else {
                if (i0 < nv) chain(pp, std::integral_constant<int, 1>{});
            }
        });
    } else if constexpr (DUAL && MAXN >= 2) {
        static_for<(MAXN + 1) / 2>([&](auto pp) {
            constexpr int i0 = 2 * decltype(pp)::value, i1 = i0 + 1;
            if constexpr (i1 < MAXN) {
                if (ng + i1 * NG < NT) two_tiles(std::integral_constant<int, i0>{}, std::integral_constant<int, i1>{});
                else if (ng + i0 * NG < NT) one_tile(std::integral_constant<int, i0>{});
            } else {
                if (ng + i0 * NG < NT) one_tile(std::integral_constant<int, i0>{});
            }
        });
    } else {
        static_for<MAXN>([&](auto ii) {
            if (ng + decltype(ii)::value * NG < NT) one_tile(ii);
        });
    }
}

struct NoHook { __device__ __forceinline__ void operator()() const {} };

template <int KQ>
struct LayerAfr {
    float4 a[KQ];
    float4 bcur;
    template <int MT>
    __device__ __forceinline__ void load(const float* wb, const LayerW& lw, int wave, int lane) {
        load_afrags<MT, KQ>(reinterpret_cast<const float4*>(wb + lw.wp), wave, lane, a);
        bcur = load_global4(wb + lw.bias + (wave % MT) * 16 + 4 * (lane >> 4));
    }
};

template <int CIN, int COUT, int V, bool RES, bool HASEMB, int T, int NB, bool FORCE = false, int CSX = cs_of(CIN), class H1, class H2>
__device__ __forceinline__ void layer_generic(const float* wb, const LayerW lw, const MixCoef<CIN, V, T, NB>& mc,
                                              const float* __restrict__ in, float* __restrict__ z, float* __restrict__ out,
                                              const float* __restrict__ embl, int wave, int lane, Prof& prof, int prof_id,
                                              H1&& pre_gemm, H2&& pre_barrier,
                                              const LayerAfr<(CIN / 16) * (RES ? 2 : 1)>* pre_afr = nullptr) {
    constexpr int MT = ceil16(COUT) / 16;
    constexpr int COLS = NB * T * V;
    constexpr int NT = ceil16(COLS) / 16;
    constexpr int TV = T * V;
    constexpr int CSI = cs_of(CIN), CSO = cs_of(COUT);
    constexpr int KQ1 = CIN / 16, KQ2 = RES ? CIN / 16 : 0;
    float4 afr[KQ1 + KQ2];
    const int trs = 8 + 8 * ((prof_id - 32) / 3);
    prof.trace(trs + 0);
    const float* bias = wb + lw.bias;
    float4 bcur;
    if (pre_afr != nullptr) {
#pragma unroll
        for (int k = 0; k < KQ1 + KQ2; ++k) afr[k] = pre_afr->a[k];
        bcur = pre_afr->bcur;
    } else {
        load_afrags<MT, KQ1 + KQ2>(reinterpret_cast<const float4*>(wb + lw.wp), wave, lane, afr);
        bcur = load_global4(bias + (wave % MT) * 16 + 4 * (lane >> 4));
    }
    mix_stage<CIN, V, T, NB, FORCE, HASEMB>(in, CSX, mc, wb + lw.tq, wb + lw.am, wave, lane,
                             ZeroInit{},
                             [&](int n, int q, int w, ChIdx c, auto v) {
                                 float* zp = (z + (n * (T * V) * CSI + q * (V * CSI) + c.cb16)) + (__mul24(w, CSI) + c.j);
                                 if constexpr (std::is_same_v<decltype(v), f32x4>) lds_store4(lds_addr(zp), v[0], v[1], v[2], v[3]);
                                 else *zp = v;
                             });
    prof.trace(trs + 1);
    pre_gemm();
    bsync();
    prof.trace(trs + 2);
    prof.mark(prof_id);
    const float slope = lw.slope;
    const float pinf = prelu_bound(slope);
    constexpr int TILE_STEP = Tiling<MT, NT>::NG * 16;
    constexpr bool FOLD = RES;
    unsigned oaddr = 0, eaddr = 0;
    auto set_bases = [&](int mi) {
        const int mt = (wave + mi * NWAVES) % MT, ng = MT > NWAVES ? 0 : wave / MT;
        const int c0 = mt * 16 + 4 * (lane >> 4);
        oaddr = lds_addr(out) + 4u * (unsigned)(__mul24(ng * 16 + (lane & 15), CSO) + c0);
        eaddr = HASEMB ? lds_addr(embl) + 4u * (unsigned)c0 : 0u;
        asm volatile("" : "+v"(oaddr), "+v"(eaddr));
    };
    set_bases(0);
    constexpr bool EHOIST = HASEMB && NB == 1 && FORCE;
    float4 e_pre = make_float4(0.f, 0.f, 0.f, 0.f);
    if constexpr (EHOIST) e_pre = lds_load4(eaddr);
    auto emb_of = [&](auto ti, int col, int ng) -> float4 {
        if constexpr (NB == 2) {
            const int tile_lo = (ng + decltype(ti)::value * Tiling<MT, NT>::NG) * 16;
            unsigned eo = tile_lo >= TV ? 4u * EMB_STRIDE : 0u;
            if (tile_lo < TV && tile_lo + 16 > TV) {
                eo = col >= TV ? 4u * EMB_STRIDE : 0u;
                asm volatile("" : "+v"(eo));
            }
            return lds_load4(eaddr + eo);
        } else if constexpr (NB > 2) {
            const int n = col / TV;
            return lds_load4(eaddr + 4u * (unsigned)((n < NB ? n : NB - 1) * EMB_STRIDE));
        } else if constexpr (EHOIST) {
            return e_pre;
        } else {
            return lds_load4(eaddr);
        }
    };
    constexpr bool EPRE = HASEMB && NB > 1 && FORCE;
    auto epi = [&](auto ti, int col, int c0, f32x4 acc, int, int ng, auto... pe) {
        if (COUT % 16 == 0 || c0 < COUT) {
            float4 e = make_float4(0.f, 0.f, 0.f, 0.f);
            if constexpr (sizeof...(pe) > 0) e = (pe, ...);
            else if constexpr (HASEMB) e = emb_of(ti, col, ng);
            f32x2 t0 = f32x2{acc[0], acc[1]}, t1 = f32x2{acc[2], acc[3]};
            if constexpr (!FOLD) { t0 += f32x2{bcur.x, bcur.y}; t1 += f32x2{bcur.z, bcur.w}; }
            const f32x2 m0 = t0 * slope, m1 = t1 * slope;
            const f32x2 r0 = f32x2{__builtin_amdgcn_fmed3f(t0[0], m0[0], pinf), __builtin_amdgcn_fmed3f(t0[1], m0[1], pinf)} + f32x2{e.x, e.y};
            const f32x2 r1 = f32x2{__builtin_amdgcn_fmed3f(t1[0], m1[0], pinf), __builtin_amdgcn_fmed3f(t1[1], m1[1], pinf)} + f32x2{e.z, e.w};
            constexpr unsigned tile_bytes = 4u * decltype(ti)::value * TILE_STEP * CSO;
            lds_store4(oaddr + tile_bytes, r0[0], r0[1], r1[0], r1[1]);
        }
    };
    prof.trace(trs + 3);
    if constexpr (EPRE) gemm_tiles<MT, NT, KQ1, KQ2, !RES, FORCE>(afr, z, CSI, in, CSX, wave, lane, epi, 0, FOLD ? bcur : make_float4(0.f, 0.f, 0.f, 0.f), emb_of);
    else gemm_tiles<MT, NT, KQ1, KQ2, !RES, FORCE>(afr, z, CSI, in, CSX, wave, lane, epi, 0, FOLD ? bcur : make_float4(0.f, 0.f, 0.f, 0.f));
#pragma unroll
    for (int mi = 1; mi < Tiling<MT, NT>::MW; ++mi) {
        load_afrags<MT, KQ1 + KQ2>(reinterpret_cast<const float4*>(wb + lw.wp), wave, lane, afr, mi);
        bcur = load_global4(bias + ((wave + mi * NWAVES) % MT) * 16 + 4 * (lane >> 4));
        set_bases(mi);
        if constexpr (EHOIST) e_pre = lds_load4(eaddr);
        if constexpr (EPRE) gemm_tiles<MT, NT, KQ1, KQ2, !RES, FORCE>(afr, z, CSI, in, CSX, wave, lane, epi, mi, FOLD ? bcur : make_float4(0.f, 0.f, 0.f, 0.f), emb_of);
        else gemm_tiles<MT, NT, KQ1, KQ2, !RES, FORCE>(afr, z, CSI, in, CSX, wave, lane, epi, mi, FOLD ? bcur : make_float4(0.f, 0.f, 0.f, 0.f));
    }
    prof.trace(trs + 4);
    pre_barrier();
#ifdef MCD_PROFILE
    asm volatile("s_waitcnt lgkmcnt(0)" ::: "memory");
#endif
    prof.trace(trs + 5);
    bsync();
    prof.trace(trs + 6);
    prof.mark(prof_id + 1);
}
template <int CIN, int COUT, int V, bool RES, bool HASEMB, int T, int NB>
__device__ __forceinline__ void layer_generic(const float* wb, const LayerW lw, const float* __restrict__ in,
                                              float* __restrict__ z, float* __restrict__ out,
                                              const float* __restrict__ embl, int wave, int lane, Prof& prof, int prof_id) {
    MixCoef<CIN, V, T, NB> mc;
    mc.load(wb + lw.tq, wb + lw.am, wave, lane);
    layer_generic<CIN, COUT, V, RES, HASEMB, T, NB>(wb, lw, mc, in, z, out, embl, wave, lane, prof, prof_id, NoHook{}, NoHook{});
}

template <int L, int T, int NB>
using LMix = MixCoef<layer_desc(L).cin, layer_desc(L).V, T, NB>;
template <int L>
using LAfr = LayerAfr<(layer_desc(L).cin / 16) * (layer_desc(L).res ? 2 : 1)>;
template <int L>
__device__ __forceinline__ void load_lafr(LAfr<L>& A, const float* wb, int wave, int lane) {
    A.template load<ceil16(layer_desc(L).cout) / 16>(wb, layer_w(wb, L), wave, lane);
}
template <int L, int T, int NB, bool FORCE = false, int CSX = cs_of(layer_desc(L).cin), class H1, class H2>
__device__ __forceinline__ void layer_std(const float* wb, const LMix<L, T, NB>& mc, const float* in, float* z, float* out,
                                          const float* emb, int wave, int lane, Prof& prof, H1&& pre_gemm, H2&& pre_barrier,
                                          const LAfr<L>* pre_afr = nullptr) {
    constexpr LDesc D = layer_desc(L);
    layer_generic<D.cin, D.cout, D.V, D.res != 0, true, T, NB, FORCE, CSX>(wb, layer_w(wb, L), mc, in, z, out, emb + emb_off(L), wave, lane,
                                                               prof, 32 + 3 * L, pre_gemm, pre_barrier, pre_afr);
}

struct EmbRow {
    float4 w[4];
    float b;
    __device__ __forceinline__ void load(const float* wb, int o) {
        const float* we = wb + tab_i(wb, TAB_WE);
#pragma unroll
        for (int q = 0; q < 4; ++q) w[q] = load_global4(we + o * EDIM + 4 * q);
        b = as_global(wb + tab_i(wb, TAB_BE))[o];
    }
};
template <int NB>
__device__ __forceinline__ void emb_row(const EmbRow& f, int o, const float* __restrict__ se, float* __restrict__ emb,
                                        float* __restrict__ e10) {
#pragma unroll
    for (int n = 0; n < NB; ++n) {
        f32x2 acc = {f.b, 0.f};
#pragma unroll
        for (int q = 0; q < 4; ++q) {
            const float4 sv = *reinterpret_cast<const float4*>(se + n * EDIM + 4 * q);
            acc = f32x2{f.w[q].x, f.w[q].y} * f32x2{sv.x, sv.y} + acc;
            acc = f32x2{f.w[q].z, f.w[q].w} * f32x2{sv.z, sv.w} + acc;
        }
        const float r = acc[0] + acc[1];
        if (o < emb_off(10)) emb[n * EMB_STRIDE + o] = r;
        else if (o < EMB_TOTAL) e10[n * 4 + (o - emb_off(10))] = r;
    }
}
constexpr int EMB_EXTRA = EMB_TOTAL > NTHREADS ? EMB_TOTAL - NTHREADS : 0;
template <int NB>
__device__ __forceinline__ void emb_compute(const EmbRow& f, const float* __restrict__ exw, const float* __restrict__ se,
                                            float* __restrict__ emb, float* __restrict__ e10, int tid) {
    static_assert(EMB_TOTAL <= 2 * NTHREADS, "two rows per thread cover the embedding outputs");
    emb_row<NB>(f, tid, se, emb, e10);
    if (tid < EMB_EXTRA) {
        EmbRow f2;
#pragma unroll
        for (int q = 0; q < 4; ++q) f2.w[q] = *reinterpret_cast<const float4*>(exw + tid * 20 + 4 * q);
        f2.b = exw[tid * 20 + 16];
        emb_row<NB>(f2, tid + NTHREADS, se, emb, e10);
    }
}

template <int T, int NB>
struct Plan {
    static constexpr int NBT = NB * T;
    static constexpr int P17 = ceil16(NBT * 17), P12 = ceil16(NBT * 12), P10 = ceil16(NBT * 10);
    static constexpr int s16 = P17 * 20, s32a = P17 * 36, s32b = P12 * 36, s64b = P12 * 68, s64c = P10 * 68, s128 = P10 * 132;
    static constexpr int L0_in = 0, L0_z = s16, L0_out = 2 * s16;
    static constexpr int L1_in = 2 * s16, L1_z = 0, L1_out = 3 * s16;
    static constexpr int L2_in = 3 * s16, L2_z = 0, L2_out = 3 * s16 + s32a;
    static constexpr int DN1_out = 0;
    static constexpr int L3_in = 0, L3_z = s32b, L3_out = 2 * s32b;
    static constexpr int L4_in = 2 * s32b, L4_z = 2 * s32b + s64b, L4_out = 0;
    static constexpr int DN2_out = s128 + s64c;
    static constexpr int L5_in = s128 + s64c, L5_z = s128, L5_out = 0;
    static constexpr int L6_in = 0, L6_p = s128;
    static constexpr int UP3_out = 0;
    static constexpr int L7_in = 0, L7_z = s64b, L7_out = 2 * s64b;
    static constexpr int L8_in = 2 * s64b, L8_z = 0, L8_out = s64b;
    static constexpr int L8_p = 0;
    static constexpr int UP2_out = cmax(s64b + s32b, 2 * s32a);
    static constexpr int L9_in = UP2_out, L9_z = 0, L9_out = s32a;
    static constexpr int L10_in = s32a, L10_p = 2 * s32a;
    static constexpr int R = cmax(cmax(cmax(s128 + 2 * s64c, 2 * s128), cmax(3 * s16 + 2 * s32a, 2 * s32b + 2 * s64b)),
                                  cmax(cmax(3 * s64b, 3 * s32a), UP2_out + s32a));
    static_assert(s32a <= 3 * s16 && s64b <= 2 * s32b && s32a <= s64b && s64b <= s128, "LDS plan: regions would overlap");
    static constexpr int XT = P17 * 4;
    static constexpr int EMB = NB * EMB_STRIDE;
    static constexpr int EAUX = 2 * 4 * 4 + 4 * EDIM;
    static constexpr int ZN = P17 * 2;
    static constexpr int WM = 12;
    static constexpr int BIA = 64 + 16 + 32;
    static constexpr int UPD = 16;
    static constexpr int ZO = P17 * 2;
    static constexpr int TT = P17 * 2;
    static constexpr int CE = 4 * EDIM;
    static constexpr int LOSS = NB * 64;
    static constexpr int EXW = EMB_EXTRA * 20;
#ifdef MCD_PROFILE
    static constexpr int PROFTR = (NB * T >= 10 && NWAVES <= 12) ? PROF_TRACE * PROF_NW : 0;
    static constexpr int PROF = PROF_SLOTS + PROFTR;
#else
    static constexpr int PROF = 0;
#endif
    static constexpr int TOTAL = R + XT + EMB + EAUX + ZN + WM + BIA + UPD + ZO + TT + CE + LOSS + EXW + PROF;
    static_assert((size_t)TOTAL * 4 <= 160 * 1024, "LDS plan: more than 160 KB");
    static constexpr size_t BYTES = (size_t)TOTAL * 4;
};

struct FrameIdx { int idx[MCD_MAX_FRAMES]; };
struct FrameMaps { int src_frame[MCD_MAX_FRAMES], tx_of[MCD_MAX_FRAMES], pos_of[MCD_MAX_FRAMES], upd_of[MCD_MAX_FRAMES]; };
__device__ __forceinline__ float loss_elem(float a, float b, int fn) {
    const float d = fabsf(a - b);
    if (fn == MCD_LOSS_SMOOTH_L1) return d < 1.f ? 0.5f * d * d : d - 0.5f;
    if (fn == MCD_LOSS_L1) return d;
    return d * d;
}

}
```

### mocodad_amd/csrc/mcd_score_kernel.hpp

```cpp
#pragma once
#include "mcd_device.hpp"

namespace mcd {

constexpr int TABC = 128;
constexpr int TABC_LW = 40, TABC_LB = 41;

template <int T, int NB, class FrameOf>
__device__ __forceinline__ void cond_fast_body(const float* wbuf, const DataView& dv, FrameOf&& frame_of, int seg_len, float* smem,
                                               int b0, int B, float* emb_lds, float* __restrict__ emb_out) {
    constexpr int P17 = ceil16(NB * T * 17);
    constexpr int s16 = P17 * 20, s32 = P17 * 36;
    constexpr int TV = T * 17, COLS = NB * TV;
    float* const X0 = smem;
    float* const Z0 = smem + s16;
    float* const Y0 = smem + 2 * s16;
    float* const Z1 = smem + 2 * s16 + s32;
    float* const H = smem;
    const int tid = threadIdx.x, lane = tid & 63;
    const int wave = __builtin_amdgcn_readfirstlane(tid >> 6);
    Prof prof;
    prof.off();
    for (int u = tid; u < COLS * C0; u += NTHREADS) {
        const int c = u % C0, col = u / C0;
        const int n = col / TV, t = (col / 17) % T, v = col % 17;
        const int b = b0 + n < B ? b0 + n : B - 1;
        X0[col * 20 + c] = load_coord(dv, b, c, frame_of(t), v, seg_len);
    }
    bsync();
    const float* wb = wbuf;
    auto lw = [&](int l) {
        LayerW w;
        w.tq = tab_i(wb, TABC + l * F_STRIDE + F_TQ); w.am = tab_i(wb, TABC + l * F_STRIDE + F_AM);
        w.wp = tab_i(wb, TABC + l * F_STRIDE + F_WP); w.bias = tab_i(wb, TABC + l * F_STRIDE + F_BIAS);
        w.slope = tab_f(wb, TABC + l * F_STRIDE + F_SLOPE);
        return w;
    };
    layer_generic<16, 32, 17, true, false, T, NB>(wb, lw(0), X0, Z0, Y0, nullptr, wave, lane, prof, 0);
    layer_generic<32, 16, 17, true, false, T, NB>(wb, lw(1), Y0, Z1, X0, nullptr, wave, lane, prof, 0);
    layer_generic<16, 32, 17, true, false, T, NB>(wb, lw(2), X0, Z0, Y0, nullptr, wave, lane, prof, 0);
    layer_generic<32, 32, 17, false, false, T, NB>(wb, lw(3), Y0, Z1, H, nullptr, wave, lane, prof, 0);
    constexpr int F = 32 * TV;
    gfloat* W = as_global(wb + tab_i(wb, TABC + TABC_LW));
    gfloat* bb = as_global(wb + tab_i(wb, TABC + TABC_LB));
    for (int u = tid; u < NB * EDIM * 16; u += NTHREADS) {
        const int part = u & 15, jo = (u >> 4) % EDIM, n = u / (16 * EDIM);
        constexpr int NT16 = (TV + 15) / 16;
        float a = 0.f;
        gfloat* wr = W + jo * F + part;
        const float* hr = H + (n * TV + part) * 36;
#pragma unroll 4
        for (int c = 0; c < 32; ++c) {
            float wv[NT16];
#pragma unroll
            for (int i = 0; i < NT16; ++i) wv[i] = (i * 16 + part < TV) ? wr[c * TV + i * 16] : 0.f;
#pragma unroll
            for (int i = 0; i < NT16; ++i) a = fmaf(wv[i], (i * 16 + part < TV) ? hr[i * 16 * 36 + c] : 0.f, a);
        }
        a = row16_sum(a);
        if (part == 0) {
            const float e = a + bb[jo];
            if (emb_lds) emb_lds[n * EDIM + jo] = e;
            if (emb_out && b0 + n < B) emb_out[(size_t)(b0 + n) * EDIM + jo] = e;
        }
    }
}

template <int T, int NB>
__global__ __launch_bounds__(NTHREADS, 2) void cond_fast_kernel(const float* wbuf, const DataView dv, const FrameIdx fi,
                                                                int seg_len, float* __restrict__ emb_out, int B) {
    constexpr int P17 = ceil16(NB * T * 17);
    extern __shared__ __attribute__((aligned(16))) float smem[];
    for (int u = threadIdx.x; u < P17 * (2 * 20 + 2 * 36); u += NTHREADS) smem[u] = 0.f;
    __syncthreads();
    cond_fast_body<T, NB>(wbuf, dv, [&](int t) { return fi.idx[t]; }, seg_len, smem, blockIdx.x * NB, B, nullptr, emb_out);
}

template <int T, int NB, int MINW, bool LT = false>
__global__ __launch_bounds__(NTHREADS, MINW) void score_kernel(const ScoreParams P) {
    using PL = Plan<T, NB>;
    constexpr int TV17 = T * 17;
    constexpr int COLS17 = NB * TV17;
    extern __shared__ __attribute__((aligned(16))) float smem[];
    float* const RG = smem;
    float* const XT = RG + PL::R;
    float* const EMB = XT + PL::XT;
    float* const E10 = EMB + PL::EMB;
    float* const SEN = E10 + 32;
    float* const ZN = E10 + PL::EAUX;
    int* const WM = reinterpret_cast<int*>(ZN + PL::ZN);
    float* const BIA = reinterpret_cast<float*>(WM + PL::WM);
    int* const UPD = reinterpret_cast<int*>(BIA + PL::BIA);
    float* const ZO = reinterpret_cast<float*>(UPD + PL::UPD);

    const int tid0 = threadIdx.x;
    int tid = tid0;
    int lane = tid & 63;
    int wave = __builtin_amdgcn_readfirstlane(tid >> 6);
    Prof prof;
    prof.off();
#ifdef MCD_PROFILE
    const unsigned long long wg_t0 = __builtin_amdgcn_s_memrealtime();
#endif
    if (P.phase > 0 && blockIdx.x * 2 >= gridDim.x) {
        const unsigned long long t0 = __builtin_readcyclecounter();
        while (__builtin_readcyclecounter() - t0 < (unsigned long long)P.phase * 1024ull) __builtin_amdgcn_s_sleep(32);
    }
    if (P.phase < -15) {
        const unsigned h = (blockIdx.x * 2654435761u) >> 26;
        const unsigned long long t0 = __builtin_readcyclecounter();
        while (__builtin_readcyclecounter() - t0 < (unsigned long long)h * (unsigned long long)(-P.phase) * 16ull) __builtin_amdgcn_s_sleep(32);
    }
    const int grp = blockIdx.x / P.split, part = blockIdx.x - grp * P.split;
    const int win0 = grp * NB;
    const int Tx = P.n_corrupt;
    auto window_of = [&](int n) { const int b = win0 + n; return b < P.B ? b : P.B - 1; };
    if (threadIdx.x < NB) {
        const int b = window_of(threadIdx.x);
        WM[threadIdx.x] = P.win_mask ? P.win_mask[b] : (int)P.fixed_mask;
        WM[4 + threadIdx.x] = b;
        if (threadIdx.x == 0) { WM[8] = 0; WM[9] = -1; }
    }
    if (threadIdx.x >= 128 && threadIdx.x < 128 + NB * T) {
        const int i = threadIdx.x - 128, n = i / T, t = i % T;
        const int fixed = P.win_mask ? P.win_mask[window_of(n)] : (int)P.fixed_mask;
        const int k = P.win_mask ? (((fixed >> t) & 1) ? -1 : 0) : P.upd_of[t];
        UPD[i] = k < 0 ? -1 : (n * T + (P.win_mask ? t : P.pos_of[k])) * 17;
    }
    static_assert(NB <= 4 && T <= 16 && NB * T <= 16, "tail index packing: 4 bits (chain, frame) | 2 bits chain | 4 bits frame");
    int* const TT = reinterpret_cast<int*>(ZO + PL::ZO);
    float* const CE = reinterpret_cast<float*>(TT + PL::TT);
    float* const LOSSB = CE + PL::CE;
    float* const EXW = LOSSB + PL::LOSS;
    if constexpr (MINW >= 4) {
        if (threadIdx.x == 0) {
            int sh = P.prio_shift;
            if (sh > 0 && P.tune) {
                const int sig = (int)gridDim.x * 1009 + P.S * 31 + P.ns;
                const int ticks = P.tune[1];
                if (P.tune[0] == sig && ticks > 0) {
                    const unsigned v = (unsigned)(((unsigned long long)(unsigned)ticks * (unsigned)(P.prio_rounds > 0 ? P.prio_rounds : 1)) / 6u) | 1u;
                    sh = 31 - __clz((int)v);
                    if ((v >> (sh > 0 ? sh - 1 : 0)) & 1u) ++sh;
                    sh = sh < 10 ? 10 : (sh > 26 ? 26 : sh);
                }
            }
            UPD[15] = sh;
            UPD[14] = (int)(unsigned)__builtin_amdgcn_s_memrealtime();
        }
    }
    for (int u = threadIdx.x; u < EMB_EXTRA * 17; u += NTHREADS) {
        const int r = u / 17, k = u % 17;
        EXW[r * 20 + k] = k < 16 ? P.wbuf[tab_i(P.wbuf, TAB_WE) + (NTHREADS + r) * EDIM + k] : P.wbuf[tab_i(P.wbuf, TAB_BE) + NTHREADS + r];
    }
    for (int u = threadIdx.x; u < COLS17 * C0; u += NTHREADS) {
        const int col = u / C0, n = col / TV17, t = (col / 17) % T, v = col % 17;
        TT[u] = (n * T + t) | (n << 4) | (t << 6) | (v << 10);
    }
    if (threadIdx.x < 64) BIA[threadIdx.x] = P.wbuf[tab_i(P.wbuf, 6 * F_STRIDE + F_BIAS) + threadIdx.x];
    else if (threadIdx.x < 64 + C0) BIA[threadIdx.x] = P.wbuf[tab_i(P.wbuf, 10 * F_STRIDE + F_BIAS) + threadIdx.x - 64];
    else if (threadIdx.x >= 80 && threadIdx.x < 112) BIA[threadIdx.x] = P.wbuf[tab_i(P.wbuf, 8 * F_STRIDE + F_BIAS) + threadIdx.x - 80];
    const int CTV = C0 * Tx * 17;
    const int K = P.ns > 2 ? P.ns - 1 : 1;

    if (P.cond_inkernel) {
        for (int u = tid; u < PL::R; u += NTHREADS) smem[u] = 0.f;
        bsync();
        cond_fast_body<T, NB>(P.wbuf, P.dv, [&](int t) { return P.cond_idx[t]; }, P.seg_len, smem, win0, P.B, CE, nullptr);
        bsync();
    } else if (threadIdx.x < NB * EDIM) {
        CE[threadIdx.x] = P.cond_emb ? P.cond_emb[(size_t)window_of(threadIdx.x / EDIM) * EDIM + threadIdx.x % EDIM] : 0.f;
    }
    for (int u = tid; u < PL::R + PL::XT; u += NTHREADS) smem[u] = 0.f;
    bsync();

#ifdef MCD_PROFILE
    prof.acc = reinterpret_cast<unsigned*>(EXW + PL::EXW);
    for (int i = tid0; i < PROF_SLOTS; i += NTHREADS) prof.acc[i] = 0u;
    prof.on = (tid0 == 0 && blockIdx.x == 0 && P.prof != nullptr); prof.tlast = __builtin_readcyclecounter();
    prof.won = ((tid0 & 63) == 0 && blockIdx.x == 0 && P.prof != nullptr); prof.wv = tid0 >> 6;
    prof.tr = (P.prof && PL::PROFTR) ? prof.acc + PROF_SLOTS : nullptr;
    for (int i = tid0; i < PL::PROFTR; i += NTHREADS) prof.acc[PROF_SLOTS + i] = 0u;
    __syncthreads();
#endif
    auto lt_inject = [&](int id, float* region, int cs, int C, int V) {
        if constexpr (LT) {
            if (P.lt_stage == id) {
                bsync();
                for (int u = threadIdx.x; u < NB * C * T * V; u += NTHREADS) {
                    const int v = u % V, t = (u / V) % T, c = (u / (V * T)) % C, n = u / (V * T * C);
                    const int b = window_of(n);
                    region[((n * T + t) * V + v) * cs + c] = P.lt_in[(((size_t)b * C + c) * T + t) * V + v];
                }
                bsync();
            }
        }
    };
    auto lt_dump = [&](int id, const float* region, int cs, int C, int V) {
        if constexpr (LT) {
            if (P.lt_stage == id) {
                bsync();
                for (int u = threadIdx.x; u < NB * C * T * V; u += NTHREADS) {
                    const int v = u % V, t = (u / V) % T, c = (u / (V * T)) % C, n = u / (V * T * C);
                    const int b = win0 + n;
                    if (b < P.B) P.lt_out[(((size_t)b * C + c) * T + t) * V + v] = region[((n * T + t) * V + v) * cs + c];
                }
                bsync();
            }
        }
    };
    using RS1 = RsCfg<32, 17, 12, T, NB, true>;
    using RS2 = RsCfg<64, 12, 10, T, NB, true>;
    float skip1[RS1::PER * RS1::SK];
    float skip2[RS2::PER * RS2::SK];
    constexpr bool LOWO = MINW <= (NWAVES == 12 ? 3 : 2);

    const int i_first = P.mode == 1 ? P.step_single : P.ns - 1;
    const int i_last = P.mode == 1 ? P.step_single : 1;
    auto silu_row = [&](int step, int t_id) {
        if (t_id >= 0 && t_id < NB * EDIM) {
            const int solo = NB > 1 ? WM[9] : -1;
            const float e = P.step_table[step * (4 + EDIM) + 4 + (t_id % EDIM)] + ((solo >= 0 && t_id / EDIM != solo) ? 0.f : CE[t_id]);
            SEN[t_id] = e / (1.f + expf(-e));
        }
    };
    for (int s = part; s < P.S; s += P.split) {
    typedef const ScoreParams __attribute__((address_space(4))) KScoreParams;
    KScoreParams* Q = (KScoreParams*)__builtin_amdgcn_kernarg_segment_ptr();
    asm volatile("" : "+s"(Q));
    int tid_s = tid0;
    asm volatile("" : "+v"(tid_s));
    {
        DataView dv;
        dv.data = Q->dv.data; dv.base = Q->dv.base; dv.sc = Q->dv.sc; dv.st = Q->dv.st; dv.trans = Q->dv.trans; dv.aff = Q->dv.aff;
        const float* noise = Q->noise;
        const float* x_in = Q->x_in;
        const int mode = Q->mode, seg_len = Q->seg_len, Bq = Q->B;
        const unsigned long long seed = Q->seed;
        const long long first_window = Q->first_window;
        for (int u = tid_s; u < COLS17; u += NTHREADS) {
            const int n = u / TV17, t = (u / 17) % T, v = u % 17;
            const int b = WM[4 + n];
            const int fixed = WM[n];
            const int solo = NB > 1 ? WM[9] : -1;
            float xv[C0];
#pragma unroll
            for (int c = 0; c < C0; ++c) {
                if (solo >= 0 && n != solo) {
                    xv[c] = 0.f;
                } else if (mode == 1) {
                    xv[c] = x_in ? x_in[((b * C0 + c) * T + t) * 17 + v] : 0.f;
                } else if ((fixed >> t) & 1) {
                    xv[c] = load_coord(dv, b, c, fm_src(P, t), v, seg_len);
                } else {
                    const int e = (c * Tx + fm_tx(P, fixed, t)) * 17 + v;
                    if (noise) xv[c] = noise[((size_t)(s * K + 0) * Bq + b) * CTV + e];
                    else xv[c] = philox_normal(seed, (unsigned)e, 0u, (unsigned)s, (unsigned)(first_window + b));
                }
            }
            XT[u * 4 + 0] = xv[0];
            XT[u * 4 + 1] = xv[1];
        }
    }
    bsync();
    {
        EmbRow er;
        er.load(P.wbuf, tid_s);
        silu_row(i_first, tid_s);
        bsync();
        emb_compute<NB>(er, EXW, SEN, EMB, E10 + (i_first & 1) * 16, tid_s);
        bsync();
    }
    LMix<0, T, NB> mc0;
    mc0.load(P.wbuf + tab_i(P.wbuf, F_TQ), P.wbuf + tab_i(P.wbuf, F_AM), wave, lane);
    constexpr bool WEARLY = T <= 4;
    LAfr<0> A0;
    if constexpr (WEARLY) load_lafr<0>(A0, P.wbuf, wave, lane);
    for (int sidx = i_first; sidx >= i_last; --sidx) {
        const float* srow = P.step_table + sidx * (4 + EDIM);
        const float* wb = P.wbuf;
        asm volatile("" : "+s"(wb));
        tid = tid0;
        asm volatile("" : "+v"(tid));
        lane = tid & 63;
        wave = __builtin_amdgcn_readfirstlane(tid >> 6);
        if constexpr (MINW >= 4) {
            const int sh = UPD[15];
            if (sh > 0) {
                unsigned hwid;
                asm volatile("s_getreg_b32 %0, hwreg(HW_REG_HW_ID)" : "=s"(hwid));
                const unsigned slice = (unsigned)(__builtin_amdgcn_s_memrealtime() >> sh);
                if (((hwid >> 16) ^ slice) & 1u) __builtin_amdgcn_s_setprio(1);
                else __builtin_amdgcn_s_setprio(0);
            }
        }
        constexpr bool NZ_TAIL = MixCfg<16, 17, T, NB>::UNITS <= NWAVES - 2;
        constexpr int NZ_T0 = NZ_TAIL ? NTHREADS - 128 : 0;
        constexpr int NZ_GROUPS = NB * T * 9;
        static_assert(NZ_GROUPS <= 128, "noise groups fit the two idle waves");
        auto noise_part = [&](int t_id) {
            const int gi = t_id - NZ_T0;
            if (P.mode == 0 && sidx > 1 && gi >= 0 && gi < NZ_GROUPS) {
                const int n = gi / (T * 9), r = gi % (T * 9), t = r / 9, v0 = (r % 9) * 2;
                float z[4] = {0.f, 0.f, 0.f, 0.f};
                const int fixed = WM[n];
                const int solo = NB > 1 ? WM[9] : -1;
                if (!((fixed >> t) & 1) && (solo < 0 || n == solo)) {
                    const int b = WM[4 + n];
                    const int tx = fm_tx(P, fixed, t);
                    const int k = P.ns - sidx;
                    if (P.noise) {
                        const float* zp = P.noise + ((size_t)(s * K + k) * P.B + b) * CTV + tx * 17 + v0;
                        z[0] = zp[0]; z[1] = zp[Tx * 17];
                        if (v0 + 1 < 17) { z[2] = zp[1]; z[3] = zp[Tx * 17 + 1]; }
                    } else {
                        philox_normal4(P.seed, (unsigned)(tx * 9 + (v0 >> 1)), (unsigned)k, (unsigned)s, (unsigned)(P.first_window + b), z);
                    }
                }
                float* zo = ZN + ((n * T + t) * 17 + v0) * C0;
                zo[0] = z[0]; zo[1] = z[1];
                if (v0 + 1 < 17) { zo[2] = z[2]; zo[3] = z[3]; }
            }
        };
        noise_part(tid);
        STAGE(0);
        STAGE(1);
#ifdef MCD_PROFILE
        prof.bidx = 0;
        prof.tr_on = prof.won && prof.tr && s == part && sidx == i_first - 1;
        prof.trace(0);
#endif
        auto mixload = [&](auto& mc, int l) { mc.load(wb + tab_i(wb, l * F_STRIDE + F_TQ), wb + tab_i(wb, l * F_STRIDE + F_AM), wave, lane); };
        auto rsload = [&](auto& rc, int r) { rc.load(wb + tab_i(wb, TAB_RSW + r), wb + tab_i(wb, TAB_RSB + r), lane); };
        auto mix_early = mixload;
        auto rs_early = rsload;
        NoHook nohook;
        constexpr bool EARLY2 = LOWO || T == 6;
        LMix<1, T, NB> mc1;
        LAfr<1> A1; LAfr<2> A2; LAfr<3> A3; LAfr<4> A4; LAfr<5> A5; LAfr<7> A7; LAfr<9> A9;
        auto wearly = [&](auto& A, auto lc) { if constexpr (WEARLY) load_lafr<decltype(lc)::value>(A, wb, wave, lane); };
#define MCD_LC(l) std::integral_constant<int, l>{}
        layer_std<0, T, NB, LOWO, 4>(wb, mc0, XT, RG + PL::L0_z, RG + PL::L0_out, EMB, wave, lane, prof,
                            [&] { mix_early(mc1, 1); }, [&] { wearly(A1, MCD_LC(1)); }, WEARLY ? &A0 : nullptr);
        STAGE(2);
        lt_dump(0, RG + PL::L0_out, 20, 16, 17);
        lt_inject(1, RG + PL::L1_in, 20, 16, 17);
        LMix<2, T, NB> mc2;
        silu_row(sidx > 0 ? sidx - 1 : 0, tid - NZ_T0);
        layer_std<1, T, NB, LOWO>(wb, mc1, RG + PL::L1_in, RG + PL::L1_z, RG + PL::L1_out, EMB, wave, lane, prof,
                            [&] { mix_early(mc2, 2); }, [&] { wearly(A2, MCD_LC(2)); }, WEARLY ? &A1 : nullptr);
        STAGE(3);
        lt_dump(1, RG + PL::L1_out, 36, 32, 17);
        lt_inject(2, RG + PL::L2_in, 36, 32, 17);
        RsCoef<32, 17, 12, T, NB, true> rc1;
        LMix<3, T, NB> mc3;
        layer_std<2, T, NB, LOWO>(wb, mc2, RG + PL::L2_in, RG + PL::L2_z, RG + PL::L2_out, EMB, wave, lane, prof,
                            [&] { rs_early(rc1, 0); }, [&] { if constexpr (EARLY2) mix_early(mc3, 3); }, WEARLY ? &A2 : nullptr);
        STAGE(4);
        lt_dump(2, RG + PL::L2_out, 36, 32, 17);
        lt_inject(11, RG + PL::L2_out, 36, 32, 17);
        if constexpr (!EARLY2) mix_early(mc3, 3);
        constexpr bool SQ12 = !LT && MixCfg<32, 12, T, NB>::SAMEQ;
        resample_stage<32, 17, 12, T, NB, true, false, LOWO, SQ12>(RG + PL::L2_out, 36, RG + PL::DN1_out, 36, rc1, skip1, wave, lane);
        wearly(A3, MCD_LC(3));
        bsync();
        STAGE(5);
        lt_dump(11, RG + PL::DN1_out, 36, 32, 12);
        lt_inject(3, RG + PL::L3_in, 36, 32, 12);
        LMix<4, T, NB> mc4;
        layer_std<3, T, NB, LOWO>(wb, mc3, RG + PL::L3_in, RG + PL::L3_z, RG + PL::L3_out, EMB, wave, lane, prof,
                            [&] { mix_early(mc4, 4); }, [&] { wearly(A4, MCD_LC(4)); }, WEARLY ? &A3 : nullptr);
        STAGE(6);
        lt_dump(3, RG + PL::L3_out, 68, 64, 12);
        lt_inject(4, RG + PL::L4_in, 68, 64, 12);
        RsCoef<64, 12, 10, T, NB, true> rc2;
        LMix<5, T, NB> mc5;
        layer_std<4, T, NB, LOWO>(wb, mc4, RG + PL::L4_in, RG + PL::L4_z, RG + PL::L4_out, EMB, wave, lane, prof,
                            [&] { rs_early(rc2, 1); }, [&] { if constexpr (EARLY2) mix_early(mc5, 5); }, WEARLY ? &A4 : nullptr);
        STAGE(7);
        lt_dump(4, RG + PL::L4_out, 68, 64, 12);
        lt_inject(12, RG + PL::L4_out, 68, 64, 12);
        if constexpr (!EARLY2) mix_early(mc5, 5);
        resample_stage<64, 12, 10, T, NB, true, false, LOWO>(RG + PL::L4_out, 68, RG + PL::DN2_out, 68, rc2, skip2, wave, lane);
        constexpr bool FUSE64 = RS2::ALIGNED && MixCfg<64, 10, T, NB>::QC == T && MixCfg<64, 10, T, NB>::UNITS == NWAVES;
        wearly(A5, MCD_LC(5));
        if constexpr (!FUSE64) bsync();
        STAGE(8);
        lt_dump(12, RG + PL::DN2_out, 68, 64, 10);
        lt_inject(5, RG + PL::L5_in, 68, 64, 10);
        RsCoef<64, 10, 12, T, NB, false> rc3;
        LMix<7, T, NB> mc7;
        {
            constexpr int NT = PL::P10 / 16;
            constexpr int COLS = NB * T * 10;
            const LayerW lw = layer_w(wb, 6);
            float4 afr[8];
            MixCoef<64, 10, T, NB> mc6;
            layer_std<5, T, NB, LOWO>(wb, mc5, RG + PL::L5_in, RG + PL::L5_z, RG + PL::L5_out, EMB, wave, lane, prof, nohook,
                                [&] {
                                    load_afrags<8, 8>(reinterpret_cast<const float4*>(wb + lw.wp), wave, lane, afr, 0);
                                    if constexpr (EARLY2) mc6.load(wb + lw.tq, wb + lw.am, wave, lane);
                                }, WEARLY ? &A5 : nullptr);
            STAGE(9);
            lt_dump(5, RG + PL::L5_out, 132, 128, 10);
            lt_inject(6, RG + PL::L6_in, 132, 128, 10);
            float* Pb = RG + PL::L6_p;
            if constexpr (!EARLY2) mc6.load(wb + lw.tq, wb + lw.am, wave, lane);
            auto epi6 = [&](auto ti, int col, int c0, f32x4 acc, int col0, int) {
                constexpr int STEP = Tiling<8, NT>::NG * 16 * 132;
                if (col < COLS) *reinterpret_cast<float4*>(Pb + __mul24(col0, 132) + c0 + decltype(ti)::value * STEP) = make_float4(acc[0], acc[1], acc[2], acc[3]);
            };
            gemm_tiles<8, NT, 8, 0, false, LOWO>(afr, RG + PL::L6_in, 132, RG + PL::L6_in, 132, wave, lane, epi6, 0);
#pragma unroll
            for (int mi = 1; mi < Tiling<8, NT>::MW; ++mi) {
                load_afrags<8, 8>(reinterpret_cast<const float4*>(wb + lw.wp), wave, lane, afr, mi);
                gemm_tiles<8, NT, 8, 0, false, LOWO>(afr, RG + PL::L6_in, 132, RG + PL::L6_in, 132, wave, lane, epi6, mi);
            }
            if constexpr (EARLY2) { rs_early(rc3, 2); mix_early(mc7, 7); }
            bsync();
            STAGE(10);
            const float slope6 = lw.slope;
            const float pinf6 = prelu_bound(slope6);
            mix_stage<64, 10, T, NB, LOWO, true>(Pb, 132, mc6, wb + lw.tq, wb + lw.am, wave, lane,
                                     [&](int n, int q, int w, ChIdx c) {
                                         const float* pp = (Pb + (n * (T * 10) * 132 + q * (10 * 132) + 64 + c.cb16)) + (__mul24(w, 132) + c.j);
                                         const float4 r = lds_load4(lds_addr(pp));
                                         return f32x4{r.x, r.y, r.z, r.w};
                                     },
                                     [&](int n, int q, int w, ChIdx c, f32x4 v) {
                                         const float4 b4 = lds_load4(lds_addr(BIA + c.cb16) + 4u * (unsigned)c.j);
                                         const float4 e4 = lds_load4(lds_addr(EMB + n * EMB_STRIDE + emb_off(6) + c.cb16) + 4u * (unsigned)c.j);
                                         float* pp = (Pb + (n * (T * 10) * 132 + q * (10 * 132) + 64 + c.cb16)) + (__mul24(w, 132) + c.j);
                                         const f32x2 t0 = f32x2{v[0], v[1]} + f32x2{b4.x, b4.y}, t1 = f32x2{v[2], v[3]} + f32x2{b4.z, b4.w};
                                         const f32x2 m0 = t0 * slope6, m1 = t1 * slope6;
                                         const f32x2 r0 = f32x2{__builtin_amdgcn_fmed3f(t0[0], m0[0], pinf6), __builtin_amdgcn_fmed3f(t0[1], m0[1], pinf6)} + f32x2{e4.x, e4.y};
                                         const f32x2 r1 = f32x2{__builtin_amdgcn_fmed3f(t1[0], m1[0], pinf6), __builtin_amdgcn_fmed3f(t1[1], m1[1], pinf6)} + f32x2{e4.z, e4.w};
                                         lds_store4(lds_addr(pp), r0[0], r0[1], r1[0], r1[1]);
                                     });
        }
        if constexpr (MINW == 3 || (MINW >= 4 && T >= 5)) {
            tid = tid0;
            asm volatile("" : "+v"(tid));
            lane = tid & 63;
            wave = __builtin_amdgcn_readfirstlane(tid >> 6);
        }
        if constexpr (!EARLY2) rs_early(rc3, 2);
        if constexpr (!FUSE64) bsync();
        STAGE(11);
        lt_dump(6, RG + PL::L6_p + 64, 132, 64, 10);
        lt_inject(13, RG + PL::L6_p + 64, 132, 64, 10);
        if constexpr (LT) {
            if (P.lt_stage == 13) for (float& f : skip2) f = 0.f;
            if (P.lt_stage == 14) for (float& f : skip1) f = 0.f;
        }
        if constexpr (!EARLY2) mix_early(mc7, 7);
        resample_stage<64, 10, 12, T, NB, false, true, LOWO>(RG + PL::L6_p + 64, 132, RG + PL::UP3_out, 68, rc3, skip2, wave, lane);
        wearly(A7, MCD_LC(7));
        bsync();
        STAGE(12);
        lt_dump(13, RG + PL::UP3_out, 68, 64, 12);
        lt_inject(7, RG + PL::L7_in, 68, 64, 12);
        RsCoef<32, 12, 17, T, NB, false> rc4;
        LMix<9, T, NB> mc9;
        {
            constexpr int NT = PL::P12 / 16;
            constexpr int COLS = NB * T * 12;
            const LayerW lw = layer_w(wb, 8);
            float4 afr8[4];
            MixCoef<32, 12, T, NB> mc8w;
            layer_std<7, T, NB, LOWO>(wb, mc7, RG + PL::L7_in, RG + PL::L7_z, RG + PL::L7_out, EMB, wave, lane, prof, nohook,
                                [&] {
                                    load_afrags<4, 4>(reinterpret_cast<const float4*>(wb + lw.wp), wave, lane, afr8, 0);
                                    if constexpr (EARLY2) mc8w.load(wb + lw.tq, wb + lw.am, wave, lane);
                                }, WEARLY ? &A7 : nullptr);
            STAGE(13);
            lt_dump(7, RG + PL::L7_out, 68, 64, 12);
            lt_inject(8, RG + PL::L8_in, 68, 64, 12);
            float* Pb = RG + PL::L8_p;
            if constexpr (!EARLY2) mc8w.load(wb + lw.tq, wb + lw.am, wave, lane);
            auto epi8 = [&](auto ti, int col, int c0, f32x4 acc, int col0, int) {
                constexpr int STEP = Tiling<4, NT>::NG * 16 * 68;
                if (col < COLS) *reinterpret_cast<float4*>(Pb + __mul24(col0, 68) + c0 + decltype(ti)::value * STEP) = make_float4(acc[0], acc[1], acc[2], acc[3]);
            };
            gemm_tiles<4, NT, 4, 0, false, LOWO>(afr8, RG + PL::L8_in, 68, RG + PL::L8_in, 68, wave, lane, epi8, 0);
#pragma unroll
            for (int mi = 1; mi < Tiling<4, NT>::MW; ++mi) {
                load_afrags<4, 4>(reinterpret_cast<const float4*>(wb + lw.wp), wave, lane, afr8, mi);
                gemm_tiles<4, NT, 4, 0, false, LOWO>(afr8, RG + PL::L8_in, 68, RG + PL::L8_in, 68, wave, lane, epi8, mi);
            }
            if constexpr (EARLY2) { rs_early(rc4, 3); mix_early(mc9, 9); }
            bsync();
            prof.mark(32 + 3 * 8 + 1);
            const float slope8 = lw.slope;
            const float pinf8 = prelu_bound(slope8);
            mix_stage<32, 12, T, NB, LOWO, true>(Pb, 68, mc8w, wb + lw.tq, wb + lw.am, wave, lane,
                                     [&](int n, int q, int w, ChIdx c) {
                                         const float* pp = (Pb + (n * (T * 12) * 68 + q * (12 * 68) + 32 + c.cb16)) + (__mul24(w, 68) + c.j);
                                         const float4 r = lds_load4(lds_addr(pp));
                                         return f32x4{r.x, r.y, r.z, r.w};
                                     },
                                     [&](int n, int q, int w, ChIdx c, f32x4 v) {
                                         const float4 b4 = lds_load4(lds_addr(BIA + 80 + c.cb16) + 4u * (unsigned)c.j);
                                         const float4 e4 = lds_load4(lds_addr(EMB + n * EMB_STRIDE + emb_off(8) + c.cb16) + 4u * (unsigned)c.j);
                                         float* pp = (Pb + (n * (T * 12) * 68 + q * (12 * 68) + 32 + c.cb16)) + (__mul24(w, 68) + c.j);
                                         const f32x2 t0 = f32x2{v[0], v[1]} + f32x2{b4.x, b4.y}, t1 = f32x2{v[2], v[3]} + f32x2{b4.z, b4.w};
                                         const f32x2 m0 = t0 * slope8, m1 = t1 * slope8;
                                         const f32x2 r0 = f32x2{__builtin_amdgcn_fmed3f(t0[0], m0[0], pinf8), __builtin_amdgcn_fmed3f(t0[1], m0[1], pinf8)} + f32x2{e4.x, e4.y};
                                         const f32x2 r1 = f32x2{__builtin_amdgcn_fmed3f(t1[0], m1[0], pinf8), __builtin_amdgcn_fmed3f(t1[1], m1[1], pinf8)} + f32x2{e4.z, e4.w};
                                         lds_store4(lds_addr(pp), r0[0], r0[1], r1[0], r1[1]);
                                     });
            if constexpr (!EARLY2) rs_early(rc4, 3);
            if constexpr (!SQ12) bsync();
            prof.mark(32 + 3 * 8);
            STAGE(14);
            lt_dump(8, RG + PL::L8_p + 32, 68, 32, 12);
            lt_inject(14, RG + PL::L8_p + 32, 68, 32, 12);
            if constexpr (!EARLY2) mix_early(mc9, 9);
            resample_stage<32, 12, 17, T, NB, false, true, LOWO, SQ12>(RG + PL::L8_p + 32, 68, RG + PL::UP2_out, 36, rc4, skip1, wave, lane);
        }
        wearly(A9, MCD_LC(9));
        bsync();
        STAGE(15);
        lt_dump(14, RG + PL::UP2_out, 36, 32, 17);
        lt_inject(9, RG + PL::L9_in, 36, 32, 17);
        {
            const LayerW lw = layer_w(wb, 10);
            MixCoef<16, 17, T, NB> mc10;
            EmbRow ef;
            auto ef_load = [&] { ef.load(wb, tid); };
            layer_std<9, T, NB, LOWO>(wb, mc9, RG + PL::L9_in, RG + PL::L9_z, RG + PL::L9_out, EMB, wave, lane, prof,
                                [&] {
                                    mc10.load(wb + lw.tq, wb + lw.am, wave, lane);
                                    ef_load();
                                }, nohook, WEARLY ? &A9 : nullptr);
            STAGE(16);
            lt_dump(9, RG + PL::L9_out, 36, 32, 17);
            lt_inject(10, RG + PL::L10_in, 36, 32, 17);
            const float ca = srow[0], cb = srow[1], csg = srow[2];
            float* Pb = RG + PL::L10_p;
            {
                const int r = wave & 3;
                const cfloat* w4 = (const cfloat*)(wb + lw.wp + r * 32);
                for (int cblk = wave >> 2; cblk * 64 < COLS17; cblk += NWAVES / 4) {
                    const int col = cblk * 64 + lane;
                    if (col < COLS17) {
                        const float* xp = RG + PL::L10_in + col * 36;
                        f32x2 acc2 = {0.f, 0.f};
#pragma unroll
                        for (int q = 0; q < 8; ++q) {
                            const float4 x = *reinterpret_cast<const float4*>(xp + 4 * q);
                            acc2 = f32x2{w4[4 * q + 0], w4[4 * q + 1]} * f32x2{x.x, x.y} + acc2;
                            acc2 = f32x2{w4[4 * q + 2], w4[4 * q + 3]} * f32x2{x.z, x.w} + acc2;
                        }
                        Pb[col * 20 + r] = acc2[0] + acc2[1];
                    }
                }
            }
            STAGE(18);
            emb_compute<NB>(ef, EXW, SEN, EMB, E10 + ((sidx - 1) & 1) * 16, tid);
            STAGE(19);
            bsync();
            STAGE(20);
            const float slope10 = lw.slope;
            const bool single = P.mode == 1, zadd = sidx > 1;
            const int e10_off = (sidx & 1) * 16;
            mix_stage<16, 17, T, NB, LOWO, true>(Pb, 20, mc10, wb + lw.tq, wb + lw.am, wave, lane,
                                     ZeroInit{},
                                     [&](int n, int t, int w, ChIdx c, auto val) {
                                         if constexpr (std::is_same_v<decltype(val), f32x4>) {
                                             if (c.j == 0) *reinterpret_cast<float2*>(ZO + ((n * T + t) * 17 + w) * C0) = make_float2(val[0], val[1]);
                                         } else {
                                             if (c.j < C0) ZO[((n * T + t) * 17 + w) * C0 + c.j] = val;
                                         }
                                     });
            bsync();
            constexpr int TAIL_IT = (COLS17 * C0 + NTHREADS - 1) / NTHREADS;
            float xn_t[TAIL_IT];
            int dst_t[TAIL_IT];
#pragma unroll
            for (int it = 0; it < TAIL_IT; ++it) {
                const int u = tid + it * NTHREADS;
                dst_t[it] = -1;
                xn_t[it] = 0.f;
                if (u < COLS17 * C0) {
                    const int c = u % C0, col = u / C0;
                    const int tt = TT[u];
                    const int n = (tt >> 4) & 3, t = (tt >> 6) & 15, v = tt >> 10;
                    const float x = XT[col * 4 + c];
                    const float l10 = prelu(ZO[u] + Pb[col * 20 + C0 + c] + BIA[64 + c], slope10) + E10[e10_off + n * 4 + c];
                    const float eps = l10 + x;
                    if constexpr (LT) {
                        const int b = win0 + n;
                        if (P.lt_stage == 10 && b < P.B) P.lt_out[(((size_t)b * C0 + c) * T + t) * 17 + v] = l10;
                    }
                    if (single) {
                        const int b = win0 + n;
                        if (b < P.B && P.eps_out) P.eps_out[(((size_t)b * C0 + c) * T + t) * 17 + v] = eps;
                    } else {
                        const int cbase = UPD[tt & 15];
                        if (cbase >= 0) {
                            const int colp = cbase + v;
                            const float z = zadd ? ZN[colp * C0 + c] : 0.f;
                            xn_t[it] = ca * (XT[colp * 4 + c] - cb * eps) + csg * z;
                            dst_t[it] = colp * 4 + c;
                        }
                    }
                }
            }
            if (P.upd_shift) bsync();
#pragma unroll
            for (int it = 0; it < TAIL_IT; ++it)
                if (dst_t[it] >= 0) XT[dst_t[it]] = xn_t[it];
            mc0.load(wb + tab_i(wb, F_TQ), wb + tab_i(wb, F_AM), wave, lane);
            wearly(A0, MCD_LC(0));
            STAGE(21);
            bsync();
            STAGE(17);
        }
    }
    if (P.mode == 1) break;

    float* RED = RG;
    const int per = CTV;
    {
        asm volatile("" : "+s"(Q));
        tid_s = tid0;
        asm volatile("" : "+v"(tid_s));
        DataView dv;
        dv.data = Q->dv.data; dv.base = Q->dv.base; dv.sc = Q->dv.sc; dv.st = Q->dv.st; dv.trans = Q->dv.trans; dv.aff = Q->dv.aff;
        const int seg_len = Q->seg_len, Bq = Q->B, Sq = Q->S, loss_fn = Q->loss_fn;
        float* pose_out = Q->pose_out;
        float* loss_out = Q->loss_out;
        const bool wmask = Q->win_mask != nullptr;
        for (int u = tid_s; u < NB * per; u += NTHREADS) {
            const int n = u / per, e = u % per;
            const int c = e / (Tx * 17), tx = (e / 17) % Tx, v = e % 17;
            const int solo = NB > 1 ? WM[9] : -1;
            const bool valid = win0 + n < Bq && (solo < 0 || n == solo);
            const int b = WM[4 + n];
            int tu = P.pos_of[tx];
            if (wmask) {
                const int fixed = WM[n];
                int cnt = 0;
                for (int t = 0; t < T; ++t)
                    if (!((fixed >> t) & 1)) { if (cnt == tx) tu = t; ++cnt; }
            }
            const float x0 = XT[((n * T + tu) * 17 + v) * 4 + c];
            const float gt = load_coord(dv, b, c, fm_src(P, tu), v, seg_len);
            const float d = fabsf(x0 - gt);
            float l;
            if (loss_fn == MCD_LOSS_SMOOTH_L1) l = d < 1.f ? 0.5f * d * d : d - 0.5f;
            else if (loss_fn == MCD_LOSS_L1) l = d;
            else l = d * d;
            RED[u] = l;
            if (valid && pose_out) pose_out[(size_t)(b * Sq + s) * per + e] = x0;
        }
        bsync();
        float* PART = RED + NB * per;
        if (tid_s < NB * 8) {
            const int n = tid_s >> 3, p8 = tid_s & 7;
            float sum = 0.f;
            for (int e = p8; e < per; e += 8) sum += RED[n * per + e];
            PART[tid_s] = sum;
        }
        bsync();
        if (tid_s < NB) {
            const int n = tid_s;
            float sum = 0.f;
#pragma unroll
            for (int k = 0; k < 8; ++k) sum += PART[n * 8 + k];
            const float l = sum / (float)per;
            const int solo = NB > 1 ? WM[9] : -1;
            if (solo < 0 || n == solo) {
                if (win0 + n < Bq && loss_out) loss_out[(size_t)(win0 + n) * Sq + s] = l;
                if (s < 64) LOSSB[n * 64 + s] = l;
                if (!(fabsf(l) <= 3.0e38f)) WM[8] = 1;
            }
        }
    }
    bsync();
    {
        const int div = WM[8], solo = NB > 1 ? WM[9] : -1;
        if (div) {
            for (int u = tid_s; u < PL::R + PL::XT; u += NTHREADS) smem[u] = 0.f;
            for (int u = tid_s; u < PL::ZN; u += NTHREADS) { ZN[u] = 0.f; ZO[u] = 0.f; }
        }
        if (NB > 1 && (div || solo >= 0)) {
            const int nxt = solo < 0 ? 0 : (solo + 1 < NB ? solo + 1 : -1);
            if (nxt >= 0) s -= P.split;
            bsync();
            if (tid_s == 0) { WM[8] = 0; WM[9] = nxt; }
            bsync();
        } else if (div) {
            bsync();
            if (tid_s == 0) WM[8] = 0;
        }
    }
    }
#ifdef MCD_PROFILE
    __syncthreads();
    if (P.prof && tid0 == 0 && blockIdx.x < 6000) {
        unsigned hwid;
        asm volatile("s_getreg_b32 %0, hwreg(HW_REG_HW_ID)" : "=s"(hwid));
        unsigned xcc;
        asm volatile("s_getreg_b32 %0, hwreg(HW_REG_XCC_ID)" : "=s"(xcc));
        P.prof[4096 + 3 * blockIdx.x] = wg_t0;
        P.prof[4096 + 3 * blockIdx.x + 1] = __builtin_amdgcn_s_memrealtime();
        P.prof[4096 + 3 * blockIdx.x + 2] = ((unsigned long long)(xcc & 0xf) << 32) | hwid;
    }
    if (prof.on) {
        for (int i = 0; i < PROF_SLOTS; ++i) P.prof[i] += prof.acc[i];
        for (int i = 0; i < PL::PROFTR; ++i) P.prof[PROF_SLOTS + i] = prof.acc[PROF_SLOTS + i];
    }
#endif
    int te = tid0;
    asm volatile("" : "+v"(te));
    if constexpr (MINW >= 4) {
        if (P.mode == 0 && P.tune && blockIdx.x == 0 && te == 0) {
            P.tune[1] = (int)((unsigned)__builtin_amdgcn_s_memrealtime() - (unsigned)UPD[14]);
            P.tune[0] = (int)gridDim.x * 1009 + P.S * 31 + P.ns;
        }
    }
    if (P.mode == 0 && P.loss_agg && te < NB && win0 + te < P.B)
        P.loss_agg[win0 + te] = aggregate_losses(LOSSB + te * 64, P.S, P.aggr, P.aggr_q);
}

constexpr int TABC_URS = 56;
constexpr int TABC_ULW = 60, TABC_ULB = 61;
constexpr int CU_OUT = 6;

template <int T, int NB>
struct CondUnetLds {
    using PL = Plan<T, NB>;
    static constexpr int H_OFF = 2 * PL::s128;
    static constexpr int FLOATS = cmax(PL::R, H_OFF + PL::P10 * 20);
};

template <int T, int NB>
__global__ __launch_bounds__(NTHREADS, 2) void cond_unet_kernel(const float* wbuf, const DataView dv, const FrameIdx fi,
                                                                int seg_len, float* __restrict__ emb_out, int B) {
    using PL = Plan<T, NB>;
    constexpr int TV17 = T * 17, COLS17 = NB * TV17, TV10 = T * 10;
    constexpr int H_OFF = CondUnetLds<T, NB>::H_OFF;
    extern __shared__ __attribute__((aligned(16))) float smem[];
    float* const RG = smem;
    const int tid = threadIdx.x, lane = tid & 63;
    const int wave = __builtin_amdgcn_readfirstlane(tid >> 6);
    const int b0 = blockIdx.x * NB;
    Prof prof;
    prof.off();
    for (int u = tid; u < CondUnetLds<T, NB>::FLOATS; u += NTHREADS) smem[u] = 0.f;
    __syncthreads();
    for (int u = tid; u < COLS17 * C0; u += NTHREADS) {
        const int c = u % C0, col = u / C0;
        const int n = col / TV17, t = (col / 17) % T, v = col % 17;
        const int b = b0 + n < B ? b0 + n : B - 1;
        RG[PL::L0_in + col * 20 + c] = load_coord(dv, b, c, fi.idx[t], v, seg_len);
    }
    __syncthreads();
    const float* wb = wbuf;
    auto lw = [&](int l) {
        LayerW w;
        w.tq = tab_i(wb, TABC + l * F_STRIDE + F_TQ); w.am = tab_i(wb, TABC + l * F_STRIDE + F_AM);
        w.wp = tab_i(wb, TABC + l * F_STRIDE + F_WP); w.bias = tab_i(wb, TABC + l * F_STRIDE + F_BIAS);
        w.slope = tab_f(wb, TABC + l * F_STRIDE + F_SLOPE);
        return w;
    };
    float nosk[1] = {0.f};
    layer_generic<16, 16, 17, true, false, T, NB>(wb, lw(0), RG + PL::L0_in, RG + PL::L0_z, RG + PL::L0_out, nullptr, wave, lane, prof, 0);
    layer_generic<16, 32, 17, true, false, T, NB>(wb, lw(1), RG + PL::L1_in, RG + PL::L1_z, RG + PL::L1_out, nullptr, wave, lane, prof, 0);
    layer_generic<32, 32, 17, false, false, T, NB>(wb, lw(2), RG + PL::L2_in, RG + PL::L2_z, RG + PL::L2_out, nullptr, wave, lane, prof, 0);
    {
        RsCoef<32, 17, 12, T, NB, false> rc;
        rc.load(wb + tab_i(wb, TABC + TABC_URS + 0), wb + tab_i(wb, TABC + TABC_URS + 1), lane);
        resample_stage<32, 17, 12, T, NB, false, false>(RG + PL::L2_out, 36, RG + PL::DN1_out, 36, rc, nosk, wave, lane);
        __syncthreads();
    }
    layer_generic<32, 64, 12, true, false, T, NB>(wb, lw(3), RG + PL::L3_in, RG + PL::L3_z, RG + PL::L3_out, nullptr, wave, lane, prof, 0);
    layer_generic<64, 64, 12, false, false, T, NB>(wb, lw(4), RG + PL::L4_in, RG + PL::L4_z, RG + PL::L4_out, nullptr, wave, lane, prof, 0);
    {
        RsCoef<64, 12, 10, T, NB, false> rc;
        rc.load(wb + tab_i(wb, TABC + TABC_URS + 2), wb + tab_i(wb, TABC + TABC_URS + 3), lane);
        resample_stage<64, 12, 10, T, NB, false, false>(RG + PL::L4_out, 68, RG + PL::DN2_out, 68, rc, nosk, wave, lane);
        __syncthreads();
    }
    layer_generic<64, 128, 10, true, false, T, NB>(wb, lw(5), RG + PL::L5_in, RG + PL::L5_z, RG + PL::L5_out, nullptr, wave, lane, prof, 0);
    layer_generic<128, 16, 10, true, false, T, NB>(wb, lw(6), RG + PL::L6_in, RG + PL::L6_p, RG + H_OFF, nullptr, wave, lane, prof, 0);
    constexpr int F = CU_OUT * TV10;
    const float* H = RG + H_OFF;
    gfloat* W = as_global(wb + tab_i(wb, TABC + TABC_ULW));
    gfloat* bb = as_global(wb + tab_i(wb, TABC + TABC_ULB));
    for (int u = tid; u < NB * EDIM * 16; u += NTHREADS) {
        const int part = u & 15, jo = (u >> 4) % EDIM, n = u / (16 * EDIM);
        float a = 0.f;
        constexpr int NT16 = (TV10 + 15) / 16;
#pragma unroll
        for (int c = 0; c < CU_OUT; ++c) {
            float wv[NT16];
#pragma unroll
            for (int i = 0; i < NT16; ++i) wv[i] = (i * 16 + part < TV10) ? W[jo * F + c * TV10 + i * 16 + part] : 0.f;
#pragma unroll
            for (int i = 0; i < NT16; ++i) a = fmaf(wv[i], (i * 16 + part < TV10) ? H[(n * TV10 + i * 16 + part) * 20 + c] : 0.f, a);
        }
        a = row16_sum(a);
        if (part == 0 && b0 + n < B) emb_out[(size_t)(b0 + n) * EDIM + jo] = a + bb[jo];
    }
}


}
```

Before: 491,900.

## Pair two chains in layer-0/10 mix GEMMs and reload kernel params from kernarg to cut registers

For the NB=2, T=3 case, the mix stage of layer 0 and layer 10 packs both chains into one wave's 16-lane fragment (PAIR), and the GEMM then uses a two-MFMA K step instead of four because the upper K rows are zero. A host-side check rejects packings where those rows are non-zero. Several loop-carried values (window base, seed index, solo flag, step table, params) are now re-read from LDS or the kernarg segment inside the step loop instead of being held in registers, which is meant to lower register pressure. The new lane remapping and the duplicated stores add complexity and risk of layout mistakes.

```diff
diff --git a/mocodad_amd/csrc/mcd_api.hip b/mocodad_amd/csrc/mcd_api.hip
--- a/mocodad_amd/csrc/mcd_api.hip
+++ b/mocodad_amd/csrc/mcd_api.hip
@@ -188,6 +188,7 @@
     HIP_TRY(hipSetDevice(device));
     struct Restore { int d; ~Restore() { (void)hipSetDevice(d); } } restore{prev_dev};
     *dbuf = nullptr;
+    if (buf.size() > (size_t)INT32_MAX) return fail(MCD_EINVAL, "packed weight buffer too large for its 32-bit offset table");
     hipError_t e = hipMalloc(reinterpret_cast<void**>(dbuf), buf.size() * sizeof(float));
     if (e != hipSuccess) return fail(MCD_EDEVICE, std::string("hipMalloc: ") + hipGetErrorString(e));
     e = hipMemcpy(*dbuf, buf.data(), buf.size() * sizeof(float), hipMemcpyHostToDevice);
@@ -230,6 +231,13 @@
     PackedModel m;
     int rc = pack_pose_model(tensors, n_tensors, cfg, m);
     if (rc != MCD_OK) return rc;
+    if (m.fast_unet) {
+        int32_t wp = 0;
+        memcpy(&wp, &m.buf[0 * F_STRIDE + F_WP], sizeof(wp));
+        for (int i = 0; i < 2 * 64; ++i)
+            if (m.buf[(size_t)wp + 4 * i + 2] != 0.f || m.buf[(size_t)wp + 4 * i + 3] != 0.f)
+                return fail(MCD_EINVAL, "packed layer 0: K rows 2..15 of its GEMM fragments are not zero");
+    }
     float* dbuf = nullptr;
     int* tune = nullptr;
     rc = upload_packed(m.buf, device, &dbuf, &tune);
diff --git a/mocodad_amd/csrc/mcd_device.hpp b/mocodad_amd/csrc/mcd_device.hpp
--- a/mocodad_amd/csrc/mcd_device.hpp
+++ b/mocodad_amd/csrc/mcd_device.hpp
@@ -32,6 +32,12 @@
 __device__ __forceinline__ void lds_store4(unsigned addr, float a, float b, float c, float d) {
     *(lds_f32x4*)(uintptr_t)addr = f32x4{a, b, c, d};
 }
+typedef int __attribute__((address_space(3))) lds_int;
+__device__ __forceinline__ int lds_word_here(const int* p) {
+    unsigned z = 0;
+    asm volatile("" : "+s"(z));
+    return *(lds_int*)(uintptr_t)(lds_addr(reinterpret_cast<const float*>(p)) + z);
+}
 typedef f32x4 __attribute__((address_space(1))) gf32x4_rw;
 __device__ __forceinline__ void store_global4(float* p, float4 v) {
     *(gf32x4_rw*)p = f32x4{v.x, v.y, v.z, v.w};
@@ -72,9 +78,10 @@
 constexpr int TAB_WE = 88, TAB_BE = 89;
 constexpr int TAB_RSW = 90, TAB_RSB = 94;
 typedef const int __attribute__((address_space(4))) cint;
-__device__ __forceinline__ int tab_i(const float* base, int idx) { return ((cint*)base)[idx]; }
+typedef const unsigned __attribute__((address_space(4))) cuint;
+__device__ __forceinline__ unsigned tab_i(const float* base, int idx) { return ((cuint*)base)[idx]; }
 __device__ __forceinline__ float tab_f(const float* base, int idx) { return ((cfloat*)base)[idx]; }
-struct LayerW { int tq, am, wp, bias; float slope; };
+struct LayerW { unsigned tq, am, wp, bias; float slope; };
 __device__ __forceinline__ LayerW layer_w(const float* base, int l) {
     LayerW w;
     w.tq = tab_i(base, l * F_STRIDE + F_TQ); w.am = tab_i(base, l * F_STRIDE + F_AM);
@@ -183,10 +190,12 @@
     float* lt_out;
     const float* lt_skip;
 };
-__device__ __forceinline__ int fm_tx(const ScoreParams& P, int fixed, int t) {
+template <class PP>
+__device__ __forceinline__ int fm_tx(const PP& P, int fixed, int t) {
     return P.win_mask ? __popc(~fixed & ((1 << t) - 1)) : P.tx_of[t];
 }
-__device__ __forceinline__ int fm_src(const ScoreParams& P, int t) { return P.win_mask ? t : P.src_frame[t]; }
+template <class PP>
+__device__ __forceinline__ int fm_src(const PP& P, int t) { return P.win_mask ? t : P.src_frame[t]; }
 
 __device__ __forceinline__ void philox_normal4(unsigned long long seed, unsigned c0, unsigned c1, unsigned c2, unsigned c3,
                                                float (&z)[4]) {
@@ -430,12 +439,15 @@
     __device__ __forceinline__ operator int() const { return cb16 + j; }
 };
 struct ZeroInit { __device__ __forceinline__ float operator()(int, int, int, int) const { return 0.f; } };
-template <int CIN, int V, int T, int NB, bool FORCE = false, bool SCORE = false, class Init, class Store>
+template <int CIN, int V, int T, int NB, bool FORCE = false, bool SCORE = false, bool PAIR = false, class Init, class Store>
 __device__ __forceinline__ void mix_stage(const float* __restrict__ in, int cs_in, const MixCoef<CIN, V, T, NB>& pre,
                                           const float* __restrict__ tqd, const float* __restrict__ af, int wave, int lane,
                                           Init&& init, Store&& store) {
     using M = MixCfg<CIN, V, T, NB>;
-    constexpr int KS = M::KS, KP = M::KP, MT = M::MT, CB = M::CB, QC = M::QC, NQ = M::NQ, PER = M::PER;
+    constexpr int KS = M::KS, KP = M::KP, MT = M::MT, CB = M::CB, QC = M::QC, NQ = M::NQ, PER = PAIR ? 1 : M::PER;
+    static_assert(!PAIR || (NB == 2 && CB == 1 && QC == 1 && NQ <= NWAVES && std::is_same_v<std::decay_t<Init>, ZeroInit>),
+                  "PAIR: two chains, one channel block, one frame per unit, accumulators from zero");
+    static_assert(!PAIR || (!M::SAMEQ && M::UNITS >= NQ), "PAIR: MixCoef::load must hand wave w < NQ the coefficients of frame w");
     constexpr bool XB32 = FORCE || SCORE;
     const int j = lane & 15, g = lane >> 4;
     const int voff_pair = 4 * (g & 1) + (g >> 1);
@@ -445,8 +457,9 @@
         unsigned ua = lds_addr(in) + 4u * (unsigned)(n * (T * V) * cs_in + cb * 16);
         asm volatile("" : "+s"(ua));
         const lds_float* ub = (const lds_float*)(uintptr_t)ua;
-        const lds_float* a_p = ub + (__mul24(voff_pair, cs_in) + j);
-        const lds_float* a_l = (V == 17) ? ub + j : ub + (__mul24(g, cs_in) + j);
+        const int jx = PAIR ? j + ((j >> 1) & 1) * (T * V * cs_in - 2) : j;
+        const lds_float* a_p = ub + (__mul24(voff_pair, cs_in) + jx);
+        const lds_float* a_l = (V == 17) ? ub + jx : ub + (__mul24(g, cs_in) + jx);
         static_for<KS>([&](auto si) {
             constexpr int ks = decltype(si)::value;
             constexpr int vbase = ks < KP ? 8 * (ks >> 1) + 2 * (ks & 1) : 4 * KP;
@@ -518,8 +531,8 @@
         MixCoef<CIN, V, T, NB> cur = pre;
         static_for<PER>([&](auto ri) {
             constexpr int rnd = decltype(ri)::value;
-            constexpr bool ALLW = (FORCE || SCORE) && !M::SAMEQ && M::UNITS == PER * NWAVES;
-            const int u = ALLW ? wave + rnd * NWAVES : M::unit_of(wave, rnd);
+            constexpr bool ALLW = !PAIR && (FORCE || SCORE) && !M::SAMEQ && M::UNITS == PER * NWAVES;
+            const int u = PAIR ? (wave < NQ ? wave : -1) : ALLW ? wave + rnd * NWAVES : M::unit_of(wave, rnd);
             constexpr bool SURE = ALLW;
             float xs[KS][T];
             load_x(SURE ? u : (u < 0 ? 0 : u), xs);
@@ -709,13 +722,14 @@
 }
 
 struct NoPre { static constexpr bool none = true; };
-template <int MT, int NT, int KQ1, int KQ2, bool IDRES, bool FORCE = false, bool DUAL = FORCE, class Epi, class Pre = NoPre>
+template <int MT, int NT, int KQ1, int KQ2, bool IDRES, bool FORCE = false, bool DUAL = FORCE, int KSTEP = 4, class Epi, class Pre = NoPre>
 __device__ __forceinline__ void gemm_tiles(const float4 (&a)[KQ1 + KQ2], const float* __restrict__ b1, int cs1,
                                            const float* __restrict__ b2, int cs2, int wave, int lane, Epi&& epi, int mi = 0,
                                            const float4 cinit = make_float4(0.f, 0.f, 0.f, 0.f), Pre&& pre = Pre{}) {
     constexpr bool HASPRE = !std::is_same_v<std::decay_t<Pre>, NoPre>;
     constexpr int NG = Tiling<MT, NT>::NG;
     constexpr int MAXN = Tiling<MT, NT>::MAXN;
+    static_assert(KSTEP == 4 || (KSTEP == 2 && !DUAL), "KSTEP: the one-tile form only");
     const int mt = (wave + mi * NWAVES) % MT, ng = MT > NWAVES ? 0 : wave / MT;
     if (NWAVES % MT != 0 && MT <= NWAVES && ng >= NG) return;
     const int j = lane & 15, g = lane >> 4;
@@ -751,8 +765,10 @@
             if constexpr (FORCE) __builtin_amdgcn_sched_barrier(0);
             c = __builtin_amdgcn_mfma_f32_16x16x4f32(a[kq].x, u.x, c, 0, 0, 0);
             c = __builtin_amdgcn_mfma_f32_16x16x4f32(a[kq].y, u.y, c, 0, 0, 0);
-            c = __builtin_amdgcn_mfma_f32_16x16x4f32(a[kq].z, u.z, c, 0, 0, 0);
-            c = __builtin_amdgcn_mfma_f32_16x16x4f32(a[kq].w, u.w, c, 0, 0, 0);
+            if constexpr (KSTEP == 4) {
+                c = __builtin_amdgcn_mfma_f32_16x16x4f32(a[kq].z, u.z, c, 0, 0, 0);
+                c = __builtin_amdgcn_mfma_f32_16x16x4f32(a[kq].w, u.w, c, 0, 0, 0);
+            }
         });
         if constexpr (HASPRE) epi(ii, col, c0, c, col0, ng, pe);
         else epi(ii, col, c0, c, col0, ng);
@@ -938,11 +954,20 @@
         load_afrags<MT, KQ1 + KQ2>(reinterpret_cast<const float4*>(wb + lw.wp), wave, lane, afr);
         bcur = load_global4(bias + (wave % MT) * 16 + 4 * (lane >> 4));
     }
-    mix_stage<CIN, V, T, NB, FORCE, HASEMB>(in, CSX, mc, wb + lw.tq, wb + lw.am, wave, lane,
+    constexpr bool PAIR = CSX == 4 && CIN == 16 && NB == 2 && T == 3;
+    mix_stage<CIN, V, T, NB, FORCE, HASEMB, PAIR>(in, CSX, mc, wb + lw.tq, wb + lw.am, wave, lane,
                              ZeroInit{},
                              [&](int n, int q, int w, ChIdx c, auto v) {
                                  float* zp = (z + (n * (T * V) * CSI + q * (V * CSI) + c.cb16)) + (__mul24(w, CSI) + c.j);
-                                 if constexpr (std::is_same_v<decltype(v), f32x4>) lds_store4(lds_addr(zp), v[0], v[1], v[2], v[3]);
+                                 if constexpr (PAIR) {
+                                     if constexpr (std::is_same_v<decltype(v), f32x4>) {
+                                         lds_store4(lds_addr(zp), v[0], v[1], v[2], v[3]);
+                                         lds_store4(lds_addr(zp) + 4u * (T * V * CSI), v[2], v[3], v[0], v[1]);
+                                     } else {
+                                         *zp = v;
+                                         zp[T * V * CSI + 2 - 2 * (c.j & 2)] = v;
+                                     }
+                                 } else if constexpr (std::is_same_v<decltype(v), f32x4>) lds_store4(lds_addr(zp), v[0], v[1], v[2], v[3]);
                                  else *zp = v;
                              });
     prof.trace(trs + 1);
@@ -1000,8 +1025,9 @@
         }
     };
     prof.trace(trs + 3);
+    constexpr int KSTEP = PAIR && !FORCE ? 2 : 4;
     if constexpr (EPRE) gemm_tiles<MT, NT, KQ1, KQ2, !RES, FORCE>(afr, z, CSI, in, CSX, wave, lane, epi, 0, FOLD ? bcur : make_float4(0.f, 0.f, 0.f, 0.f), emb_of);
-    else gemm_tiles<MT, NT, KQ1, KQ2, !RES, FORCE>(afr, z, CSI, in, CSX, wave, lane, epi, 0, FOLD ? bcur : make_float4(0.f, 0.f, 0.f, 0.f));
+    else gemm_tiles<MT, NT, KQ1, KQ2, !RES, FORCE, FORCE, KSTEP>(afr, z, CSI, in, CSX, wave, lane, epi, 0, FOLD ? bcur : make_float4(0.f, 0.f, 0.f, 0.f));
 #pragma unroll
     for (int mi = 1; mi < Tiling<MT, NT>::MW; ++mi) {
         load_afrags<MT, KQ1 + KQ2>(reinterpret_cast<const float4*>(wb + lw.wp), wave, lane, afr, mi);
diff --git a/mocodad_amd/csrc/mcd_score_kernel.hpp b/mocodad_amd/csrc/mcd_score_kernel.hpp
--- a/mocodad_amd/csrc/mcd_score_kernel.hpp
+++ b/mocodad_amd/csrc/mcd_score_kernel.hpp
@@ -79,6 +79,7 @@
 template <int T, int NB, int MINW, bool LT = false>
 __global__ __launch_bounds__(NTHREADS, MINW) void score_kernel(const ScoreParams P) {
     using PL = Plan<T, NB>;
+    typedef const ScoreParams __attribute__((address_space(4))) KScoreParams;
     constexpr int TV17 = T * 17;
     constexpr int COLS17 = NB * TV17;
     extern __shared__ __attribute__((aligned(16))) float smem[];
@@ -119,7 +120,7 @@
         const int b = window_of(threadIdx.x);
         WM[threadIdx.x] = P.win_mask ? P.win_mask[b] : (int)P.fixed_mask;
         WM[4 + threadIdx.x] = b;
-        if (threadIdx.x == 0) { WM[8] = 0; WM[9] = -1; }
+        if (threadIdx.x == 0) { WM[8] = 0; WM[9] = -1; WM[11] = win0; }
     }
     if (threadIdx.x >= 128 && threadIdx.x < 128 + NB * T) {
         const int i = threadIdx.x - 128, n = i / T, t = i % T;
@@ -185,12 +186,16 @@
 #endif
     auto lt_inject = [&](int id, float* region, int cs, int C, int V) {
         if constexpr (LT) {
-            if (P.lt_stage == id) {
+            KScoreParams* L = (KScoreParams*)__builtin_amdgcn_kernarg_segment_ptr();
+            asm volatile("" : "+s"(L));
+            if (L->lt_stage == id) {
                 bsync();
+                const int w0 = lds_word_here(WM + 11), Bl = L->B;
+                const float* lt_in = L->lt_in;
                 for (int u = threadIdx.x; u < NB * C * T * V; u += NTHREADS) {
                     const int v = u % V, t = (u / V) % T, c = (u / (V * T)) % C, n = u / (V * T * C);
-                    const int b = window_of(n);
-                    region[((n * T + t) * V + v) * cs + c] = P.lt_in[(((size_t)b * C + c) * T + t) * V + v];
+                    const int b = w0 + n < Bl ? w0 + n : Bl - 1;
+                    region[((n * T + t) * V + v) * cs + c] = lt_in[(((size_t)b * C + c) * T + t) * V + v];
                 }
                 bsync();
             }
@@ -198,12 +203,16 @@
     };
     auto lt_dump = [&](int id, const float* region, int cs, int C, int V) {
         if constexpr (LT) {
-            if (P.lt_stage == id) {
+            KScoreParams* L = (KScoreParams*)__builtin_amdgcn_kernarg_segment_ptr();
+            asm volatile("" : "+s"(L));
+            if (L->lt_stage == id) {
                 bsync();
+                const int w0 = lds_word_here(WM + 11), Bl = L->B;
+                float* lt_out = L->lt_out;
                 for (int u = threadIdx.x; u < NB * C * T * V; u += NTHREADS) {
                     const int v = u % V, t = (u / V) % T, c = (u / (V * T)) % C, n = u / (V * T * C);
-                    const int b = win0 + n;
-                    if (b < P.B) P.lt_out[(((size_t)b * C + c) * T + t) * V + v] = region[((n * T + t) * V + v) * cs + c];
+                    const int b = w0 + n;
+                    if (b < Bl) lt_out[(((size_t)b * C + c) * T + t) * V + v] = region[((n * T + t) * V + v) * cs + c];
                 }
                 bsync();
             }
@@ -216,20 +225,19 @@
     constexpr bool LOWO = MINW <= (NWAVES == 12 ? 3 : 2);
 
     const int i_first = P.mode == 1 ? P.step_single : P.ns - 1;
-    const int i_last = P.mode == 1 ? P.step_single : 1;
-    auto silu_row = [&](int step, int t_id) {
+    auto silu_row = [&](const float* step_table, int step, int t_id) {
         if (t_id >= 0 && t_id < NB * EDIM) {
-            const int solo = NB > 1 ? WM[9] : -1;
-            const float e = P.step_table[step * (4 + EDIM) + 4 + (t_id % EDIM)] + ((solo >= 0 && t_id / EDIM != solo) ? 0.f : CE[t_id]);
+            const int solo = NB > 1 ? lds_word_here(WM + 9) : -1;
+            const float e = step_table[step * (4 + EDIM) + 4 + (t_id % EDIM)] + ((solo >= 0 && t_id / EDIM != solo) ? 0.f : CE[t_id]);
             SEN[t_id] = e / (1.f + expf(-e));
         }
     };
     for (int s = part; s < P.S; s += P.split) {
-    typedef const ScoreParams __attribute__((address_space(4))) KScoreParams;
     KScoreParams* Q = (KScoreParams*)__builtin_amdgcn_kernarg_segment_ptr();
     asm volatile("" : "+s"(Q));
     int tid_s = tid0;
     asm volatile("" : "+v"(tid_s));
+    if (tid_s == 0) WM[10] = s;
     {
         DataView dv;
         dv.data = Q->dv.data; dv.base = Q->dv.base; dv.sc = Q->dv.sc; dv.st = Q->dv.st; dv.trans = Q->dv.trans; dv.aff = Q->dv.aff;
@@ -266,26 +274,29 @@
     {
         EmbRow er;
         er.load(P.wbuf, tid_s);
-        silu_row(i_first, tid_s);
+        silu_row(Q->step_table, i_first, tid_s);
         bsync();
         emb_compute<NB>(er, EXW, SEN, EMB, E10 + (i_first & 1) * 16, tid_s);
         bsync();
     }
+    constexpr bool PAIR2 = NB == 2 && T == 3;
     LMix<0, T, NB> mc0;
     mc0.load(P.wbuf + tab_i(P.wbuf, F_TQ), P.wbuf + tab_i(P.wbuf, F_AM), wave, lane);
     constexpr bool WEARLY = T <= 4;
     LAfr<0> A0;
     if constexpr (WEARLY) load_lafr<0>(A0, P.wbuf, wave, lane);
-    for (int sidx = i_first; sidx >= i_last; --sidx) {
-        const float* srow = P.step_table + sidx * (4 + EDIM);
-        const float* wb = P.wbuf;
+    for (int sidx = i_first;; --sidx) {
+        KScoreParams* R = (KScoreParams*)__builtin_amdgcn_kernarg_segment_ptr();
+        asm volatile("" : "+s"(R));
+        const float* srow = R->step_table + sidx * (4 + EDIM);
+        const float* wb = R->wbuf;
         asm volatile("" : "+s"(wb));
         tid = tid0;
         asm volatile("" : "+v"(tid));
         lane = tid & 63;
         wave = __builtin_amdgcn_readfirstlane(tid >> 6);
         if constexpr (MINW >= 4) {
-            const int sh = UPD[15];
+            const int sh = lds_word_here(UPD + 15);
             if (sh > 0) {
                 unsigned hwid;
                 asm volatile("s_getreg_b32 %0, hwreg(HW_REG_HW_ID)" : "=s"(hwid));
@@ -300,21 +311,23 @@
         static_assert(NZ_GROUPS <= 128, "noise groups fit the two idle waves");
         auto noise_part = [&](int t_id) {
             const int gi = t_id - NZ_T0;
-            if (P.mode == 0 && sidx > 1 && gi >= 0 && gi < NZ_GROUPS) {
+            if (R->mode == 0 && sidx > 1 && gi >= 0 && gi < NZ_GROUPS) {
                 const int n = gi / (T * 9), r = gi % (T * 9), t = r / 9, v0 = (r % 9) * 2;
                 float z[4] = {0.f, 0.f, 0.f, 0.f};
                 const int fixed = WM[n];
-                const int solo = NB > 1 ? WM[9] : -1;
+                const int solo = NB > 1 ? lds_word_here(WM + 9) : -1;
                 if (!((fixed >> t) & 1) && (solo < 0 || n == solo)) {
                     const int b = WM[4 + n];
-                    const int tx = fm_tx(P, fixed, t);
-                    const int k = P.ns - sidx;
-                    if (P.noise) {
-                        const float* zp = P.noise + ((size_t)(s * K + k) * P.B + b) * CTV + tx * 17 + v0;
-                        z[0] = zp[0]; z[1] = zp[Tx * 17];
-                        if (v0 + 1 < 17) { z[2] = zp[1]; z[3] = zp[Tx * 17 + 1]; }
+                    const int tx = fm_tx(*R, fixed, t);
+                    const int k = R->ns - sidx;
+                    const int sq = lds_word_here(WM + 10);
+                    const int Txq = R->n_corrupt, Kq = R->ns > 2 ? R->ns - 1 : 1;
+                    if (R->noise) {
+                        const float* zp = R->noise + ((size_t)(sq * Kq + k) * R->B + b) * (C0 * Txq * 17) + tx * 17 + v0;
+                        z[0] = zp[0]; z[1] = zp[Txq * 17];
+                        if (v0 + 1 < 17) { z[2] = zp[1]; z[3] = zp[Txq * 17 + 1]; }
                     } else {
-                        philox_normal4(P.seed, (unsigned)(tx * 9 + (v0 >> 1)), (unsigned)k, (unsigned)s, (unsigned)(P.first_window + b), z);
+                        philox_normal4(R->seed, (unsigned)(tx * 9 + (v0 >> 1)), (unsigned)k, (unsigned)sq, (unsigned)(R->first_window + b), z);
                     }
                 }
                 float* zo = ZN + ((n * T + t) * 17 + v0) * C0;
@@ -346,7 +359,7 @@
         lt_dump(0, RG + PL::L0_out, 20, 16, 17);
         lt_inject(1, RG + PL::L1_in, 20, 16, 17);
         LMix<2, T, NB> mc2;
-        silu_row(sidx > 0 ? sidx - 1 : 0, tid - NZ_T0);
+        silu_row(R->step_table, sidx > 0 ? sidx - 1 : 0, tid - NZ_T0);
         layer_std<1, T, NB, LOWO>(wb, mc1, RG + PL::L1_in, RG + PL::L1_z, RG + PL::L1_out, EMB, wave, lane, prof,
                             [&] { mix_early(mc2, 2); }, [&] { wearly(A2, MCD_LC(2)); }, WEARLY ? &A1 : nullptr);
         STAGE(3);
@@ -450,8 +463,8 @@
         lt_dump(6, RG + PL::L6_p + 64, 132, 64, 10);
         lt_inject(13, RG + PL::L6_p + 64, 132, 64, 10);
         if constexpr (LT) {
-            if (P.lt_stage == 13) for (float& f : skip2) f = 0.f;
-            if (P.lt_stage == 14) for (float& f : skip1) f = 0.f;
+            if (R->lt_stage == 13) for (float& f : skip2) f = 0.f;
+            if (R->lt_stage == 14) for (float& f : skip1) f = 0.f;
         }
         if constexpr (!EARLY2) mix_early(mc7, 7);
         resample_stage<64, 10, 12, T, NB, false, true, LOWO>(RG + PL::L6_p + 64, 132, RG + PL::UP3_out, 68, rc3, skip2, wave, lane);
@@ -562,13 +575,19 @@
             bsync();
             STAGE(20);
             const float slope10 = lw.slope;
-            const bool single = P.mode == 1, zadd = sidx > 1;
+            const bool single = R->mode == 1, zadd = sidx > 1;
             const int e10_off = (sidx & 1) * 16;
-            mix_stage<16, 17, T, NB, LOWO, true>(Pb, 20, mc10, wb + lw.tq, wb + lw.am, wave, lane,
+            constexpr bool PAIR10 = PAIR2;
+            mix_stage<16, 17, T, NB, LOWO, true, PAIR10>(Pb, 20, mc10, wb + lw.tq, wb + lw.am, wave, lane,
                                      ZeroInit{},
                                      [&](int n, int t, int w, ChIdx c, auto val) {
                                          if constexpr (std::is_same_v<decltype(val), f32x4>) {
-                                             if (c.j == 0) *reinterpret_cast<float2*>(ZO + ((n * T + t) * 17 + w) * C0) = make_float2(val[0], val[1]);
+                                             if (c.j == 0) {
+                                                 *reinterpret_cast<float2*>(ZO + ((n * T + t) * 17 + w) * C0) = make_float2(val[0], val[1]);
+                                                 if constexpr (PAIR10) *reinterpret_cast<float2*>(ZO + ((T + t) * 17 + w) * C0) = make_float2(val[2], val[3]);
+                                             }
+                                         } else if constexpr (PAIR10) {
+                                             if (c.j < 2 * C0) ZO[(t * 17 + w) * C0 + c.j + (c.j >> 1) * (T * 17 * C0 - C0)] = val;
                                          } else {
                                              if (c.j < C0) ZO[((n * T + t) * 17 + w) * C0 + c.j] = val;
                                          }
@@ -590,12 +609,12 @@
                     const float l10 = prelu(ZO[u] + Pb[col * 20 + C0 + c] + BIA[64 + c], slope10) + E10[e10_off + n * 4 + c];
                     const float eps = l10 + x;
                     if constexpr (LT) {
-                        const int b = win0 + n;
-                        if (P.lt_stage == 10 && b < P.B) P.lt_out[(((size_t)b * C0 + c) * T + t) * 17 + v] = l10;
+                        const int b = lds_word_here(WM + 11) + n;
+                        if (R->lt_stage == 10 && b < R->B) R->lt_out[(((size_t)b * C0 + c) * T + t) * 17 + v] = l10;
                     }
                     if (single) {
-                        const int b = win0 + n;
-                        if (b < P.B && P.eps_out) P.eps_out[(((size_t)b * C0 + c) * T + t) * 17 + v] = eps;
+                        const int b = lds_word_here(WM + 11) + n;
+                        if (b < R->B && R->eps_out) R->eps_out[(((size_t)b * C0 + c) * T + t) * 17 + v] = eps;
                     } else {
                         const int cbase = UPD[tt & 15];
                         if (cbase >= 0) {
@@ -607,7 +626,7 @@
                     }
                 }
             }
-            if (P.upd_shift) bsync();
+            if (R->upd_shift) bsync();
 #pragma unroll
             for (int it = 0; it < TAIL_IT; ++it)
                 if (dst_t[it] >= 0) XT[dst_t[it]] = xn_t[it];
@@ -617,12 +636,14 @@
             bsync();
             STAGE(17);
         }
+        if (sidx <= (R->mode == 1 ? R->step_single : 1)) break;
     }
     if (P.mode == 1) break;
 
     float* RED = RG;
     const int per = CTV;
     {
+        Q = (KScoreParams*)__builtin_amdgcn_kernarg_segment_ptr();
         asm volatile("" : "+s"(Q));
         tid_s = tid0;
         asm volatile("" : "+v"(tid_s));
```

Result: no change. 495,900 (median of 6 runs) (+0.8%).
